# fuxiao0719/PanopticNeRF

Measured on AMD Instinct MI355X. Metric: Msamples/sec (coarse+fine), KITTI-360 1408x376, higher is better.
Workload: dtype bf16

## Files before the change

### include/pnr.h

```cpp
#ifndef PNR_H
#define PNR_H
#include <stdint.h>

#ifdef __cplusplus
extern "C" {
#endif

#define PNR_OK 0
#define PNR_EINVAL (-1)
#define PNR_EHIP (-2)
#define PNR_ENODEV (-3)

#define PNR_PREC_BF16 0
#define PNR_PREC_FP32 1

int pnr_version(void);
const char* pnr_last_error(void);
int pnr_device_check(int dev, char* buf_host, int buflen);

int pnr_stratified(const float* rays, int64_t n_rays, int n_samples, int lindisp,
                   const float* t_rand, float* z_out, void* stream);

int pnr_points(const float* rays, const float* z, int64_t n_rays, int n_samples, float* pts_out,
               void* stream);

int pnr_embed(const float* x, int64_t n, int L, float* out, void* stream);

typedef struct pnr_mlp_desc {
    int32_t D, W, skip;
    int32_t xyz_L, dir_L;
    int32_t n_sem, n_inst, head_W;
    int32_t precision;
    int32_t plan;
    int32_t head_tap;
    int32_t head_depth;
    int32_t schedule;
    int32_t clk_probe[2];
    int32_t flags;
} pnr_mlp_desc;

#define PNR_MLP_SOFTMAX 1
#define PNR_MLP_WG_CAP(n) (((n) & 0x1FF) << 16)
#define PNR_MLP_TRACE 0x7A00

typedef struct pnr_mlp_params_host {
    const float* const* pts_w; const float* const* pts_b;
    const float* alpha_w; const float* alpha_b;
    const float* feature_w; const float* feature_b;
    const float* views_w; const float* views_b;
    const float* rgb_w; const float* rgb_b;
    const float* sem0_w; const float* sem0_b; const float* sem1_w; const float* sem1_b;
    const float* inst0_w; const float* inst0_b; const float* inst1_w; const float* inst1_b;
} pnr_mlp_params_host;

int64_t pnr_mlp_packed_bytes(const pnr_mlp_desc* desc);
int pnr_mlp_pack(const pnr_mlp_desc* desc, const pnr_mlp_params_host* params, void* packed_host);

int64_t pnr_mlp_pack_workspace_bytes(const pnr_mlp_desc* desc, int backward);
int pnr_mlp_pack_device(const pnr_mlp_desc* desc, const pnr_mlp_params_host* params_dev, int backward,
                        void* workspace, void* packed, void* stream);
int pnr_mlp_repack_device(const pnr_mlp_desc* desc, const pnr_mlp_params_host* params_dev, int backward,
                          void* workspace, void* packed, void* stream);

int pnr_mlp_forward(const pnr_mlp_desc* desc, const void* packed, const float* rays, const float* z,
                    int64_t n_rays, int n_samples, float* raw, int64_t raw_stride_s,
                    int64_t raw_stride_c, void* stream);

int pnr_mlp_fused_plan(const pnr_mlp_desc* desc);
int64_t pnr_mlp_forward_composite_workspace_bytes(const pnr_mlp_desc* desc, int64_t n_rays, int n_samples, int want_weights);
int pnr_mlp_forward_composite(const pnr_mlp_desc* desc, const void* packed, const float* rays, const float* z,
                              int64_t n_rays, int n_samples, const int32_t* label_sem, const int32_t* label_inst,
                              int white_bkgd, float* rgb, float* depth, float* acc, float* weights, float* sem,
                              float* inst, float* fix_sem, float* fix_inst, void* workspace, void* stream);

int pnr_mlp_forward_tiles(const pnr_mlp_desc* desc, const void* packed, const float* rays, const float* z, int64_t n_rays,
                          int n_samples, void* workspace, void* stream);
int pnr_composite_combine(const pnr_mlp_desc* desc, const void* workspace, const float* z, int64_t n_rays, int n_samples,
                          const int32_t* label_sem, const int32_t* label_inst, int white_bkgd, float* rgb, float* depth,
                          float* acc, float* weights, float* sem, float* inst, float* fix_sem, float* fix_inst, void* stream);

int pnr_mlp_query(const pnr_mlp_desc* desc, const void* packed, const float* points, int64_t n_points,
                  float* sigma, int32_t* sem_label, int32_t* inst_label, int32_t* panoptic, const int32_t* is_thing,
                  float* sem_logits, float* inst_logits, int64_t logit_stride, void* stream);
int pnr_mlp_query_supported(const pnr_mlp_desc* desc);

int pnr_mlp_train_layout(const pnr_mlp_desc* desc, int64_t n_samples, int64_t* acts_off_host ,
                         int64_t* dys_off_host );
int pnr_mlp_forward_train(const pnr_mlp_desc* desc, const void* packed, const float* rays, const float* z,
                          int64_t n_rays, int n_samples, float* raw, int64_t raw_stride_s,
                          int64_t raw_stride_c, void* acts, void* stream);
int64_t pnr_mlp_bwd_packed_bytes(const pnr_mlp_desc* desc);
int pnr_mlp_pack_bwd(const pnr_mlp_desc* desc, const pnr_mlp_params_host* params, void* packed_host);
int pnr_mlp_backward(const pnr_mlp_desc* desc, const void* packed_bwd, const float* d_raw, const void* acts,
                     void* dys, int64_t n_rays, int n_samples, void* stream);

int64_t pnr_mlp_wgrad_workspace_bytes(const pnr_mlp_desc* desc, int64_t n_samples);
int pnr_mlp_wgrad(const pnr_mlp_desc* desc, const void* acts, const void* dys, int64_t n_samples,
                  const pnr_mlp_params_host* grads_dev, void* workspace, void* stream);

int64_t pnr_mlp_fp32_acts_floats(const pnr_mlp_desc* desc, int64_t n_samples);
int64_t pnr_mlp_backward_fp32_workspace_bytes(const pnr_mlp_desc* desc, int64_t n_samples);
int pnr_mlp_forward_train_fp32(const pnr_mlp_desc* desc, const pnr_mlp_params_host* params_dev, const float* rays,
                               const float* z, int64_t n_rays, int n_samples, float* raw, int64_t raw_stride_s,
                               int64_t raw_stride_c, float* acts, void* stream);
int pnr_mlp_backward_fp32(const pnr_mlp_desc* desc, const pnr_mlp_params_host* params_dev, const float* d_raw,
                          int64_t d_raw_stride_c, const float* acts, int64_t n_rays, int n_samples,
                          const pnr_mlp_params_host* grads_dev, void* workspace, void* stream);

int pnr_composite(const float* raw, int64_t raw_stride_s, int64_t raw_stride_c, const float* z,
                  const float* rays, const float* noise, const int32_t* label_sem,
                  const int32_t* label_inst, int64_t n_rays, int n_samples, int n_sem, int n_inst,
                  int sem_mode, int white_bkgd, float* rgb, float* depth, float* acc, float* weights,
                  float* sem, float* inst, float* fix_sem, float* fix_inst, void* stream);

int pnr_composite_backward(const float* raw, int64_t raw_stride_c, const float* z, const float* rays,
                           const float* noise, int64_t n_rays, int n_samples, int n_sem, int n_inst,
                           const float* g_rgb, const float* g_depth, const float* g_acc, const float* g_sem,
                           const float* g_inst, const float* g_weights, float* d_raw, void* stream);

int pnr_composite_backward2(const float* raw, int64_t raw_stride_c, const float* z, const float* rays,
                            const float* noise, int64_t n_rays, int n_samples, int n_sem, int n_inst,
                            const float* g_rgb, const float* g_depth, const float* g_acc, const float* g_sem,
                            const float* g_inst, const float* g_weights, const int32_t* label_sem,
                            const int32_t* label_inst, const float* g_fix_sem, const float* g_fix_inst,
// ... 174 lines not shown
```

### panopticnerf_amd/_lib.py

```python
import ctypes
import os

_HERE = os.path.dirname(os.path.abspath(__file__))
LIB_PATH = os.environ.get("PNR_LIB_PATH") or os.path.join(_HERE, "libpnr.so")

c_f = ctypes.c_void_p
c_i64 = ctypes.c_int64
c_int = ctypes.c_int

PREC_BF16, PREC_FP32 = 0, 1
MLP_SOFTMAX, MLP_TRACE = 1, 0x7A00
CAMERA_PINHOLE, CAMERA_FISHEYE, CAMERA_EQUIRECT = 0, 1, 3
TAG_PIXEL, TAG_FRAME = 16, 17
SAMPLE_POOLED, SAMPLE_FRAME = 0, 1


class LossCfg(ctypes.Structure):
    _fields_ = [("w_rgb", ctypes.c_float), ("w_depth", ctypes.c_float), ("w_sem", ctypes.c_float),
                ("w_fix_sem", ctypes.c_float), ("w_inst", ctypes.c_float), ("w_fix_inst", ctypes.c_float),
                ("depth_l2", ctypes.c_int32), ("fix_eps", ctypes.c_float), ("maps_are_prob", ctypes.c_int32)]


class MlpDesc(ctypes.Structure):
    _fields_ = [("D", ctypes.c_int32), ("W", ctypes.c_int32), ("skip", ctypes.c_int32),
                ("xyz_L", ctypes.c_int32), ("dir_L", ctypes.c_int32),
                ("n_sem", ctypes.c_int32), ("n_inst", ctypes.c_int32), ("head_W", ctypes.c_int32),
                ("precision", ctypes.c_int32), ("plan", ctypes.c_int32), ("head_tap", ctypes.c_int32),
                ("head_depth", ctypes.c_int32), ("schedule", ctypes.c_int32), ("clk_probe", ctypes.c_int32 * 2), ("flags", ctypes.c_int32)]


class RngDesc(ctypes.Structure):
    _fields_ = [("call", ctypes.c_void_p), ("ray_base", ctypes.c_int64), ("tag", ctypes.c_int32), ("scale", ctypes.c_float)]


class Frame(ctypes.Structure):
    _fields_ = [("model", ctypes.c_int32), ("width", ctypes.c_int32), ("height", ctypes.c_int32), ("cam", ctypes.c_float * 7),
                ("c2w", ctypes.c_float * 12), ("near_", ctypes.c_float), ("far_", ctypes.c_float), ("n_valid", ctypes.c_int64),
                ("valid_pix", ctypes.c_uint64), ("rgb", ctypes.c_uint64), ("depth", ctypes.c_uint64), ("sem", ctypes.c_uint64),
                ("inst", ctypes.c_uint64)]


_fp = ctypes.POINTER(ctypes.c_float)
_fpp = ctypes.POINTER(_fp)


class MlpParamsHost(ctypes.Structure):
    _fields_ = [("pts_w", _fpp), ("pts_b", _fpp),
                ("alpha_w", _fp), ("alpha_b", _fp), ("feature_w", _fp), ("feature_b", _fp),
                ("views_w", _fp), ("views_b", _fp), ("rgb_w", _fp), ("rgb_b", _fp),
                ("sem0_w", _fp), ("sem0_b", _fp), ("sem1_w", _fp), ("sem1_b", _fp),
                ("inst0_w", _fp), ("inst0_b", _fp), ("inst1_w", _fp), ("inst1_b", _fp)]


SIGNATURES = {
    "pnr_version": (c_int, []),
    "pnr_last_error": (ctypes.c_char_p, []),
    "pnr_device_check": (c_int, [c_int, ctypes.c_char_p, c_int]),
    "pnr_stratified": (c_int, [c_f, c_i64, c_int, c_int, c_f, c_f, c_f]),
    "pnr_points": (c_int, [c_f, c_f, c_i64, c_int, c_f, c_f]),
    "pnr_embed": (c_int, [c_f, c_i64, c_int, c_f, c_f]),
    "pnr_mlp_packed_bytes": (c_i64, [ctypes.POINTER(MlpDesc)]),
    "pnr_mlp_pack": (c_int, [ctypes.POINTER(MlpDesc), ctypes.POINTER(MlpParamsHost), ctypes.c_void_p]),
    "pnr_mlp_pack_workspace_bytes": (c_i64, [ctypes.POINTER(MlpDesc), c_int]),
    "pnr_mlp_pack_device": (c_int, [ctypes.POINTER(MlpDesc), ctypes.POINTER(MlpParamsHost), c_int, c_f, c_f, c_f]),
    "pnr_mlp_repack_device": (c_int, [ctypes.POINTER(MlpDesc), ctypes.POINTER(MlpParamsHost), c_int, c_f, c_f, c_f]),
    "pnr_mlp_forward": (c_int, [ctypes.POINTER(MlpDesc), c_f, c_f, c_f, c_i64, c_int, c_f, c_i64, c_i64, c_f]),
    "pnr_mlp_train_layout": (c_int, [ctypes.POINTER(MlpDesc), c_i64, ctypes.POINTER(c_i64), ctypes.POINTER(c_i64)]),
    "pnr_mlp_forward_train": (c_int, [ctypes.POINTER(MlpDesc), c_f, c_f, c_f, c_i64, c_int, c_f, c_i64, c_i64, c_f, c_f]),
    "pnr_mlp_bwd_packed_bytes": (c_i64, [ctypes.POINTER(MlpDesc)]),
    "pnr_mlp_pack_bwd": (c_int, [ctypes.POINTER(MlpDesc), ctypes.POINTER(MlpParamsHost), ctypes.c_void_p]),
    "pnr_mlp_backward": (c_int, [ctypes.POINTER(MlpDesc), c_f, c_f, c_f, c_f, c_i64, c_int, c_f]),
    "pnr_mlp_wgrad_workspace_bytes": (c_i64, [ctypes.POINTER(MlpDesc), c_i64]),
    "pnr_mlp_wgrad": (c_int, [ctypes.POINTER(MlpDesc), c_f, c_f, c_i64, ctypes.POINTER(MlpParamsHost), c_f, c_f]),
    "pnr_mlp_fp32_acts_floats": (c_i64, [ctypes.POINTER(MlpDesc), c_i64]),
    "pnr_mlp_backward_fp32_workspace_bytes": (c_i64, [ctypes.POINTER(MlpDesc), c_i64]),
    "pnr_mlp_forward_train_fp32": (c_int, [ctypes.POINTER(MlpDesc), ctypes.POINTER(MlpParamsHost), c_f, c_f, c_i64, c_int, c_f, c_i64,
                                           c_i64, c_f, c_f]),
    "pnr_mlp_backward_fp32": (c_int, [ctypes.POINTER(MlpDesc), ctypes.POINTER(MlpParamsHost), c_f, c_i64, c_f, c_i64, c_int,
                                      ctypes.POINTER(MlpParamsHost), c_f, c_f]),
    "pnr_mlp_fused_plan": (c_int, [ctypes.POINTER(MlpDesc)]),
    "pnr_mlp_forward_composite_workspace_bytes": (c_i64, [ctypes.POINTER(MlpDesc), c_i64, c_int, c_int]),
    "pnr_mlp_forward_composite": (c_int, [ctypes.POINTER(MlpDesc), c_f, c_f, c_f, c_i64, c_int, c_f, c_f, c_int,
                                          c_f, c_f, c_f, c_f, c_f, c_f, c_f, c_f, c_f, c_f]),
    "pnr_composite": (c_int, [c_f, c_i64, c_i64, c_f, c_f, c_f, c_f, c_f, c_i64, c_int, c_int, c_int, c_int,
                              c_int, c_f, c_f, c_f, c_f, c_f, c_f, c_f, c_f, c_f]),
    "pnr_composite_backward": (c_int, [c_f, c_i64, c_f, c_f, c_f, c_i64, c_int, c_int, c_int,
                                       c_f, c_f, c_f, c_f, c_f, c_f, c_f, c_f]),
    "pnr_composite_backward2": (c_int, [c_f, c_i64, c_f, c_f, c_f, c_i64, c_int, c_int, c_int,
                                        c_f, c_f, c_f, c_f, c_f, c_f, c_f, c_f, c_f, c_f, c_f, c_f, c_f, c_f]),
    "pnr_composite_backward3": (c_int, [c_f, c_i64, c_f, c_f, c_f, c_i64, c_int, c_int, c_int, c_int,
                                        c_f, c_f, c_f, c_f, c_f, c_f, c_f, c_f, c_f, c_f, c_f, c_f, c_f, c_f]),
    "pnr_losses_workspace_bytes": (c_i64, [c_i64]),
    "pnr_losses": (c_int, [ctypes.POINTER(LossCfg), c_i64, c_int, c_int] + [c_f] * 19),
    "pnr_ce3d_workspace_bytes": (c_i64, [c_i64]),
# ... 83 lines not shown
```

### panopticnerf_amd/csrc/pnr_composite.hip

```cpp
#include "pnr_composite_dev.h"

struct CompositeArgs {
    const float* raw; int64_t stride_s, stride_c;
    const float* z; const float* rays; const float* noise;
    const int32_t* label_sem; const int32_t* label_inst;
    int64_t R; int N, C, K, sem_mode, white_bkgd;
    float *rgb, *depth, *acc, *weights, *sem, *inst, *fix_sem, *fix_inst;
    int use_hist;
};

#ifndef CMP_GRID_PER_CU
#define CMP_GRID_PER_CU 8
#endif
#ifndef CMP_UB
#define CMP_UB 8
#endif

__device__ __forceinline__ float dot4(const f4& w, const f4& v)
{
    return fmaf(w.v[3], v.v[3], fmaf(w.v[2], v.v[2], fmaf(w.v[1], v.v[1], w.v[0] * v.v[0])));
}

template <bool CH_MAJOR, int SUB, bool SOFTMAX, class... Rng>
__global__ __launch_bounds__(256) void k_composite(CompositeArgs a, const Rng... rng)
// ... 221 lines not shown
            group_sum_batch<L, CMP2_UB>(r);
            if (writer) store_rows<CMP2_UB>(a, ray, q0, nq, r, accv);
        }
    }
}

static int composite_impl(const float* raw, int64_t raw_stride_s, int64_t raw_stride_c, const float* z, const float* rays,
                          const float* noise, const PnrRngDev* rng, const int32_t* label_sem, const int32_t* label_inst, int64_t n_rays,
                          int n_samples, int n_sem, int n_inst, int sem_mode, int white_bkgd, float* rgb, float* depth, float* acc,
                          float* weights, float* sem, float* inst, float* fix_sem, float* fix_inst, void* stream)
{
    PNR_REQUIRE(n_rays <= 0 || (raw && z && rays), "pnr_composite: null pointer");
    PNR_REQUIRE(n_samples >= 4 && n_samples <= 256 && (n_samples % 4) == 0,
                "pnr_composite: n_samples=%d must be a multiple of 4 in [4,256]", n_samples);
    PNR_REQUIRE(n_sem >= 0 && n_inst >= 0 && (sem_mode == 0 || sem_mode == 1), "pnr_composite: bad field sizes");
    PNR_REQUIRE((((uintptr_t)z) & 15) == 0, "pnr_composite: z must be 16-byte aligned");
    PNR_REQUIRE(!weights || (((uintptr_t)weights) & 15) == 0, "pnr_composite: weights must be 16-byte aligned");
    PNR_REQUIRE((((uintptr_t)noise) & 15) == 0 && (((uintptr_t)label_sem) & 15) == 0 && (((uintptr_t)label_inst) & 15) == 0,
                "pnr_composite: noise / label arrays must be 16-byte aligned");
    if (n_rays <= 0) return PNR_OK;
    CompositeArgs a;
    a.raw = raw; a.stride_s = raw_stride_s; a.stride_c = raw_stride_c; a.z = z; a.rays = rays; a.noise = noise;
    a.label_sem = label_sem; a.label_inst = label_inst; a.R = n_rays; a.N = n_samples; a.C = n_sem; a.K = n_inst;
    a.sem_mode = sem_mode; a.white_bkgd = white_bkgd; a.rgb = rgb; a.depth = depth; a.acc = acc; a.weights = weights;
    a.sem = sem; a.inst = inst; a.fix_sem = fix_sem; a.fix_inst = fix_inst;
    const bool want_fix = (fix_sem && label_sem && n_sem) || (fix_inst && label_inst && n_inst);
    const bool ch_major = raw_stride_s == 1 && (raw_stride_c % 4) == 0 && (((uintptr_t)raw) & 15) == 0;
    hipStream_t st = (hipStream_t)stream;
    auto hist_bytes = [&](int rpw) { return (size_t)4 * rpw * (n_sem + n_inst) * sizeof(uint32_t); };
    auto grid_for = [&](int rpw) { return pnr_grid_cap(((n_rays + rpw - 1) / rpw + 3) / 4, CMP_GRID_PER_CU); };
    if (ch_major && n_samples > 32 && n_samples <= 64 && (!want_fix || hist_bytes(8) <= 48 * 1024)) {
        a.use_hist = want_fix ? 1 : 0;
        const size_t lds = want_fix ? hist_bytes(8) : 0;
        composite_dispatch<8>(8, true, sem_mode, rng, [&](auto L, auto, auto SM, const auto&... r) {
            hipLaunchKernelGGL((k_composite2<decltype(L)::value, 2, decltype(SM)::value, std::decay_t<decltype(r)>...>), dim3(grid_for(8)), dim3(256),
                               lds, st, a, r...);
        });
        PNR_CHECK_LAUNCH("pnr_composite");
        return PNR_OK;
    }
    int sub = 1;
    while (sub < n_samples / 4) sub <<= 1;
    const int rpw = 64 / sub;
    a.use_hist = (want_fix && hist_bytes(rpw) <= 48 * 1024) ? 1 : 0;
    const size_t lds = a.use_hist ? hist_bytes(rpw) : 0;
    composite_dispatch<1, 2, 4, 8, 16, 32, 64>(sub, ch_major, sem_mode, rng, [&](auto S, auto CH, auto SM, const auto&... r) {
        hipLaunchKernelGGL((k_composite<decltype(CH)::value, decltype(S)::value, decltype(SM)::value, std::decay_t<decltype(r)>...>),
                           dim3(grid_for(rpw)), dim3(256), lds, st, a, r...);
    });
    PNR_CHECK_LAUNCH("pnr_composite");
    return PNR_OK;
}

PNR_EXPORT int pnr_composite(const float* raw, int64_t raw_stride_s, int64_t raw_stride_c, const float* z,
                             const float* rays, const float* noise, const int32_t* label_sem,
                             const int32_t* label_inst, int64_t n_rays, int n_samples, int n_sem, int n_inst,
                             int sem_mode, int white_bkgd, float* rgb, float* depth, float* acc, float* weights,
                             float* sem, float* inst, float* fix_sem, float* fix_inst, void* stream)
{
    return composite_impl(raw, raw_stride_s, raw_stride_c, z, rays, noise, nullptr, label_sem, label_inst, n_rays, n_samples, n_sem, n_inst,
                          sem_mode, white_bkgd, rgb, depth, acc, weights, sem, inst, fix_sem, fix_inst, stream);
}

PNR_EXPORT int pnr_composite_rng(const float* raw, int64_t raw_stride_s, int64_t raw_stride_c, const float* z, const float* rays,
                                 const pnr_rng* noise_host, const int32_t* label_sem, const int32_t* label_inst, int64_t n_rays,
                                 int n_samples, int n_sem, int n_inst, int sem_mode, int white_bkgd, float* rgb, float* depth, float* acc,
                                 float* weights, float* sem, float* inst, float* fix_sem, float* fix_inst, void* stream)
{
    PnrRngDev rng;
    const int rc = pnr_rng_check(noise_host, n_rays < 0 ? 0 : n_rays, "pnr_composite_rng", &rng);
    if (rc) return rc;
    PNR_REQUIRE(n_rays <= 0 || (raw_stride_s == 1 && (raw_stride_c % 4) == 0 && (((uintptr_t)raw) & 15) == 0),
                "pnr_composite_rng: channel-major, 16-byte aligned raw images only");
    return composite_impl(raw, raw_stride_s, raw_stride_c, z, rays, nullptr, &rng, label_sem, label_inst, n_rays, n_samples, n_sem, n_inst,
                          sem_mode, white_bkgd, rgb, depth, acc, weights, sem, inst, fix_sem, fix_inst, stream);
}

struct CombineArgs {
    const float* rec; int rec_floats; const float4* ps; const float* z; const int32_t* lab_s; const int32_t* lab_i;
    int64_t R; int N, C, K, white_bkgd;
    float *rgb, *depth, *acc, *weights, *sem, *inst, *fix_sem, *fix_inst;
};

template <bool LOGITS>
__global__ __launch_bounds__(256) void k_composite_combine(CombineArgs a)
{
    __shared__ uint32_t hist_all[4][128];
    const int lane = threadIdx.x & 63, wv = threadIdx.x >> 6;
    const int64_t ray = ((int64_t)blockIdx.x * blockDim.x + threadIdx.x) >> 6;
    if (ray >= a.R) return;
    const int N = a.N, T = N >> 5, RF = a.rec_floats, C = a.C, K = a.K, CK = C + K;
    const float* __restrict__ rec = a.rec + ray * T * RF;
    const float4* __restrict__ ps = a.ps + ray * N;
    const float* __restrict__ zr = a.z + ray * N;
    const bool want_s = a.lab_s && a.fix_sem && C, want_i = a.lab_i && a.fix_inst && K;
    const int32_t* __restrict__ lsr = want_s ? a.lab_s + ray * N : nullptr;
    const int32_t* __restrict__ lir = want_i ? a.lab_i + ray * N : nullptr;
    float q[8];
#pragma unroll
    for (int k = 0; k < 8; ++k) q[k] = k < T ? rec[k * RF] : 1.0f;
    float4 pv[4];
    float zv[4];
    int lsv[4], liv[4];
#pragma unroll
    for (int j = 0; j < 4; ++j) {
        const int i = lane + 64 * j;
        const bool in = i < N;
        pv[j] = in ? ps[i] : float4{0.0f, 0.0f, 0.0f, 0.0f};
        zv[j] = in ? zr[i] : 0.0f;
        lsv[j] = (in && want_s) ? lsr[i] : -1;
        liv[j] = (in && want_i) ? lir[i] : -1;
    }
    float lg[2][8];
#pragma unroll
    for (int h = 0; h < 2; ++h)
#pragma unroll
        for (int k = 0; k < 8; ++k) lg[h][k] = (LOGITS && k < T && lane + 64 * h < CK) ? rec[k * RF + PNR_FUSE_REC_LOGITS + lane + 64 * h] : 0.0f;
    float Tk[8];
    float t = 1.0f;
#pragma unroll
    for (int k = 0; k < 8; ++k) {
        Tk[k] = t;
        if (k < T) t *= q[k];
    }
    uint32_t* hist = hist_all[wv];
    if (want_s || want_i) hist_zero<64>(hist, lane, CK);
    float r5[5] = {0.0f, 0.0f, 0.0f, 0.0f, 0.0f};
#pragma unroll
    for (int j = 0; j < 4; ++j) {
        const int i = lane + 64 * j;
        if (i < N) {
            const float4 p = pv[j];
            float tk = Tk[0];
#pragma unroll
            for (int k = 1; k < 8; ++k) tk = (i >> 5) == k ? Tk[k] : tk;
            const float w = tk * p.x;
            r5[0] += w;
            r5[1] = fmaf(w, zv[j], r5[1]);
            r5[2] = fmaf(w, sigmoid_of(p.y), r5[2]);
            r5[3] = fmaf(w, sigmoid_of(p.z), r5[3]);
            r5[4] = fmaf(w, sigmoid_of(p.w), r5[4]);
            if (a.weights) a.weights[ray * N + i] = w;
            if (want_s || want_i) hist_add(hist, w, want_s, lsv[j], C, want_i, liv[j], K);
        }
    }
    group_sum_batch<64, 5>(r5);
    if (lane == 0) {
        if (a.acc) a.acc[ray] = r5[0];
        if (a.depth) a.depth[ray] = r5[1];
    }
    if (lane < 3 && a.rgb) {
        const float v = lane == 0 ? r5[2] : lane == 1 ? r5[3] : r5[4];
        a.rgb[ray * 3 + lane] = a.white_bkgd ? v + (1.0f - r5[0]) : v;
    }
#pragma unroll
    for (int h = 0; h < 2; ++h) {
        const int c = lane + 64 * h;
        if (c >= CK) continue;
        if constexpr (LOGITS) {
            float v = 0.0f;
#pragma unroll
            for (int k = 0; k < 8; ++k) if (k < T) v = fmaf(Tk[k], lg[h][k], v);
            if (c < C) { if (a.sem) a.sem[ray * C + c] = v; }
            else if (a.inst) a.inst[ray * K + (c - C)] = v;
        }
        if (c < C) { if (want_s) a.fix_sem[ray * C + c] = hist_read(hist, c); }
        else if (want_i) a.fix_inst[ray * K + (c - C)] = hist_read(hist, c);
    }
}

int pnr_composite_combine_launch(const float* rec, int rec_floats, bool logit_sums, const float4* ps, const float* z,
                                 const int32_t* label_sem, const int32_t* label_inst, int64_t R, int N, int C, int K, int white_bkgd,
                                 float* rgb, float* depth, float* acc, float* weights, float* sem, float* inst, float* fix_sem,
                                 float* fix_inst, hipStream_t st)
{
    CombineArgs a;
    a.rec = rec; a.rec_floats = rec_floats; a.ps = ps; a.z = z; a.lab_s = label_sem; a.lab_i = label_inst;
    a.R = R; a.N = N; a.C = C; a.K = K; a.white_bkgd = white_bkgd;
    a.rgb = rgb; a.depth = depth; a.acc = acc; a.weights = weights; a.sem = sem; a.inst = inst; a.fix_sem = fix_sem; a.fix_inst = fix_inst;
    const int64_t blocks = (R + 3) / 4;
    if (logit_sums) hipLaunchKernelGGL(k_composite_combine<true>, dim3((unsigned)blocks), dim3(256), 0, st, a);
    else hipLaunchKernelGGL(k_composite_combine<false>, dim3((unsigned)blocks), dim3(256), 0, st, a);
    PNR_CHECK_LAUNCH("pnr_mlp_forward_composite (combine)");
    return PNR_OK;
}
```

### panopticnerf_amd/csrc/pnr_mlp.hip

```cpp
#include <stdlib.h>
#include <string.h>

#include "pnr_mlp_plan.h"

int pnr_mlp_validate(const pnr_mlp_desc* d);

#include "pnr_mlp_core.h"
#include "pnr_mlp_pp.h"
#ifndef PNR_FUSE_TRANSPOSED
#define PNR_FUSE_TRANSPOSED 1
#endif
#include "pnr_mlp_fuse.h"
#include "pnr_mlp_tt.h"
#define PNR_QUERY_MAX_POINTS (((int64_t)1 << 31) - 4096)
#ifndef PNR_TRAIN_TILES_EXPERIMENT
#define PNR_TRAIN_TILES_EXPERIMENT 0
#endif
template <int PREC, int TILES, class CTX, int KIND, int NA, int NB, int NFB_OUT, int MODE, int NOUT>
__device__ __forceinline__ void layer_regs(CTX& c, const uint32_t (&inA)[TILES][NA],
                                           const uint32_t (&inB)[TILES][NB > 0 ? NB : 1],
                                           uint32_t (&out)[TILES][NOUT], uint16_t* save = nullptr,
                                           const int* srow = nullptr)
{
    constexpr int RPB = PrecT<PREC>::RPB;
// ... 717 lines not shown
    return PNR_OK;
}


static inline unsigned long long* clk_probe_of(const pnr_mlp_desc* d)
{
    return (unsigned long long*)(uintptr_t)(((uint64_t)(uint32_t)d->clk_probe[1] << 32) | (uint64_t)(uint32_t)d->clk_probe[0]);
}

static void mlp_args_fill(MlpArgs& a, const pnr_mlp_desc* desc, const PnrPlan& plan, const void* packed)
{
    memset(&a, 0, sizeof(a));
    a.data = (const uint8_t*)packed + plan.data_off;
    a.table = (const pnr_chunk_entry*)((const uint8_t*)packed + plan.table_off);
    a.n_chunks = (int)plan.chunks.size();
    a.slot_bytes = plan.max_chunk_frags * PNR_FRAG_BYTES;
    a.D = desc->D; a.skip = desc->skip; a.n_sem = desc->n_sem; a.n_inst = desc->n_inst;
    a.head_tap = desc->head_tap; a.head_depth = desc->head_depth == 1 ? 1 : 2;
    a.clk = clk_probe_of(desc);
#if PNR_TRACE
    if (const char* e = getenv("PNR_TRACE_PTR")) a.trace = (unsigned long long*)strtoull(e, nullptr, 0);
#endif
}

static int mlp_forward_impl(const pnr_mlp_desc* desc, const void* packed, const float* rays, const float* z,
                            int64_t n_rays, int n_samples, float* raw, int64_t raw_stride_s, int64_t raw_stride_c,
                            void* acts, void* stream)
{
    int rc = pnr_mlp_validate(desc);
    if (rc != PNR_OK) return rc;
    PNR_REQUIRE(n_rays >= 0 && n_samples >= 1, "pnr_mlp_forward: bad size");
    if (n_rays == 0) return PNR_OK;
    PNR_REQUIRE(packed && rays && z && raw, "pnr_mlp_forward: null pointer");
    PNR_REQUIRE(n_rays * (int64_t)n_samples < ((int64_t)1 << 31) - 4096, "pnr_mlp_forward: R*N=%lld exceeds 2^31",
                (long long)(n_rays * n_samples));
    PNR_REQUIRE((((uintptr_t)rays) & 15) == 0 && (((uintptr_t)packed) & 15) == 0 && (((uintptr_t)acts) & 15) == 0,
                "pnr_mlp_forward: rays / packed / acts must be 16-byte aligned");
    PNR_REQUIRE(!acts || desc->precision == PNR_PREC_BF16, "pnr_mlp_forward_train: the training path is bf16 only");
    PNR_REQUIRE(desc->plan != 4, "pnr_mlp_forward: a plan-4 (field) image is for pnr_mlp_query only");
    PNR_REQUIRE(desc->plan == 0, "pnr_mlp_forward: plan=%d images are for pnr_mlp_forward_composite only", desc->plan);
    PnrPlan plan;
    pnr_build_plan(*desc, plan);
    MlpArgs a;
    mlp_args_fill(a, desc, plan, packed);
    a.rays = rays; a.z = z; a.S = (int)(n_rays * n_samples); a.N = n_samples;
    pnr_set_div_magic(n_samples, a.n_magic, a.n_shift);
    a.raw = raw; a.ss = raw_stride_s; a.sc = raw_stride_c;
    a.acts = (uint16_t*)acts;
    if (acts) pnr_train_layout(*desc, a.S, a.acts_off, a.dys_off, a.gate_off);
    hipStream_t st = (hipStream_t)stream;
    if (desc->precision == PNR_PREC_BF16) {
        if (desc->schedule != 1 && !acts)
            return desc->W == 256 ? launch_mlp_pp<256, false>(a, st) : launch_mlp_pp<128, false>(a, st);
        if (desc->schedule == 2 && acts)
            return desc->W == 256 ? launch_mlp_pp<256, true>(a, st) : launch_mlp_pp<128, true>(a, st);
#if PNR_TRAIN_TILES_EXPERIMENT
        if (acts && desc->schedule == 3 && desc->W == 256) return launch_mlp<PNR_PREC_BF16, 256, 2, 4, 1, true>(a, st);
        if (acts && desc->schedule == 4 && desc->W == 256) {
            PNR_REQUIRE(a.S % 384 == 0, "schedule 4 (experiment): S must be a multiple of 384");
            return launch_mlp<PNR_PREC_BF16, 256, 3, 4, 1, true>(a, st);
        }
#endif
        if (acts)
            return desc->W == 256 ? launch_mlp<PNR_PREC_BF16, 256, 1, 8, 2, true>(a, st)
                                  : launch_mlp<PNR_PREC_BF16, 128, 1, 8, 2, true>(a, st);
        return desc->W == 256 ? launch_mlp<PNR_PREC_BF16, 256, 1, 8, 2>(a, st) : launch_mlp<PNR_PREC_BF16, 128, 1, 8, 2>(a, st);
    }
    return desc->W == 256 ? launch_mlp<PNR_PREC_FP32, 256, 1, 4, 1>(a, st) : launch_mlp<PNR_PREC_FP32, 128, 1, 4, 1>(a, st);
}

PNR_EXPORT int pnr_mlp_forward(const pnr_mlp_desc* desc, const void* packed, const float* rays, const float* z,
                               int64_t n_rays, int n_samples, float* raw, int64_t raw_stride_s,
                               int64_t raw_stride_c, void* stream)
{
    return mlp_forward_impl(desc, packed, rays, z, n_rays, n_samples, raw, raw_stride_s, raw_stride_c, nullptr, stream);
}

#define PNR_RAY_AUX_BYTES 128
#define PNR_TT_SAVE_REGION (352 * 1024)
static bool pnr_tt_save_proto() { static const bool on = getenv("PNR_TT_SAVE_PROTO") != nullptr; return on; }
int pnr_composite_combine_launch(const float* rec, int rec_floats, bool logit_sums, const float4* ps, const float* z,
                                 const int32_t* label_sem, const int32_t* label_inst, int64_t R, int N, int C, int K, int white_bkgd,
                                 float* rgb, float* depth, float* acc, float* weights, float* sem, float* inst, float* fix_sem,
                                 float* fix_inst, hipStream_t st);

static int record_floats(const pnr_mlp_desc& d)
{
    return d.plan == 3 ? pnr_fuse_record_floats(0, 0) : pnr_fuse_record_floats(d.n_sem, d.n_inst);
}

PNR_EXPORT int64_t pnr_mlp_forward_composite_workspace_bytes(const pnr_mlp_desc* desc, int64_t n_rays, int n_samples, int want_weights)
{
    (void)want_weights;
    if (pnr_mlp_validate(desc) != PNR_OK || n_rays < 0 || n_samples < 32 || (n_samples & 31)) return -1;
    const int64_t S = n_rays * n_samples, tiles = (S + 255) / 256 * 8;
    if (desc->plan == 3) return tiles * record_floats(*desc) * 4 + S * 16 + 256;
    return tiles * pnr_fuse_record_floats(desc->n_sem, desc->n_inst) * 4 + S * 16 + 256 + PNR_RAY_AUX_BYTES + n_rays * PNR_RAY_AUX_BYTES +
           (pnr_tt_save_proto() ? tiles / 8 * 4 * PNR_TT_SAVE_REGION + 4096 : 0);
}

__global__ void __launch_bounds__(256) k_ray_aux(const float* __restrict__ rays, int64_t R, uint32_t* __restrict__ aux)
{
    const int64_t i = (int64_t)blockIdx.x * 256 + threadIdx.x;
    if (i >= 2 * R) return;
    const int64_t ray = i >> 1;
    const int hi = (int)(i & 1);
    const float dx = rays[ray * 8 + 3], dy = rays[ray * 8 + 4], dz = rays[ray * 8 + 5];
    const float nrm = sqrtf(__fadd_rn(__fadd_rn(__fmul_rn(dx, dx), __fmul_rn(dy, dy)), __fmul_rn(dz, dz)));
    uint32_t ed[8];
    embed_lane<PNR_PREC_BF16, 2, 16, 8>(dx / nrm, dy / nrm, dz / nrm, hi, ed);
    uint4* o = reinterpret_cast<uint4*>(aux + i * 16);
    o[0] = make_uint4(ed[0], ed[1], ed[2], ed[3]);
    o[1] = make_uint4(ed[4], ed[5], ed[6], ed[7]);
    o[2] = make_uint4(__float_as_uint(nrm), 0u, 0u, 0u);
}

static int fused_mlp_launch(const pnr_mlp_desc* desc, const void* packed, const float* rays, const float* z, int64_t n_rays,
                            int n_samples, void* workspace, void* stream, MlpArgs& a)
{
    int rc = pnr_mlp_validate(desc);
    if (rc != PNR_OK) return rc;
    PNR_REQUIRE(desc->precision == PNR_PREC_BF16, "pnr_mlp_forward_composite: bf16 only");
    PNR_REQUIRE(desc->plan != 4, "pnr_mlp_forward_composite: a plan-4 (field) image is for pnr_mlp_query only");
    PNR_REQUIRE(n_rays >= 1 && n_samples >= 32 && n_samples <= 256 && (n_samples & 31) == 0,
                "pnr_mlp_forward_composite: n_samples=%d must be a multiple of 32 in [32,256]", n_samples);
    PNR_REQUIRE(desc->n_sem + desc->n_inst <= 128, "pnr_mlp_forward_composite: n_sem + n_inst <= 128");
    PNR_REQUIRE(packed && rays && z && workspace, "pnr_mlp_forward_composite: null pointer");
    PNR_REQUIRE(n_rays * (int64_t)n_samples < ((int64_t)1 << 31) - 4096, "pnr_mlp_forward_composite: R*N exceeds 2^31");
    PNR_REQUIRE((((uintptr_t)rays | (uintptr_t)packed | (uintptr_t)workspace) & 15) == 0,
                "pnr_mlp_forward_composite: rays / packed / workspace must be 16-byte aligned");
    PnrPlan plan;
    pnr_build_plan(*desc, plan);
    mlp_args_fill(a, desc, plan, packed);
    a.rays = rays; a.z = z; a.S = (int)(n_rays * n_samples); a.N = n_samples;
    pnr_set_div_magic(n_samples, a.n_magic, a.n_shift);
    a.rec_floats = record_floats(*desc);
    a.rec = (float*)workspace;
    const int64_t tiles = ((int64_t)a.S + 255) / 256 * 8;
    a.ps = (float4*)(a.rec + tiles * a.rec_floats);
    hipStream_t st = (hipStream_t)stream;
    const bool softmax = (desc->flags & PNR_MLP_SOFTMAX) && desc->n_sem + desc->n_inst > 0;
    if (desc->plan == 3)
        return desc->W == 256 ? launch_mlp_pp<256, false, true, 0, true>(a, st) : launch_mlp_pp<128, false, true, 0, true>(a, st);
    if (desc->plan == 2) {
        PnrTTArgs t;
        memset(&t, 0, sizeof(t));
        t.image = a.data; t.rays = rays; t.z = z; t.S = a.S; t.N = a.N; t.n_magic = a.n_magic; t.n_shift = a.n_shift;
        t.rec = a.rec; t.rec_floats = a.rec_floats; t.ps = a.ps; t.n_sem = a.n_sem; t.n_inst = a.n_inst; t.clk = a.clk;
        PNR_REQUIRE(n_rays < ((int64_t)1 << 24), "pnr_mlp_forward_composite: the two-tile kernel addresses 2^24 rays per launch");
        uint32_t* aux = (uint32_t*)(((uintptr_t)((uint8_t*)a.ps + (int64_t)a.S * 16 + 256) + PNR_RAY_AUX_BYTES - 1)
                                    & ~(uintptr_t)(PNR_RAY_AUX_BYTES - 1));
        k_ray_aux<<<dim3((unsigned)((2 * n_rays + 255) / 256)), dim3(256), 0, st>>>(rays, n_rays, aux);
        t.aux = aux;
        t.n_wg = (desc->flags >> 16) & 0x1FF;
        if (pnr_tt_save_proto()) t.save = (void*)(((uintptr_t)((uint8_t*)aux + n_rays * PNR_RAY_AUX_BYTES) + 4095) & ~(uintptr_t)4095);
        const bool trace = (desc->flags & 0xFF00) == PNR_MLP_TRACE;
        return pnr_mlp_tt_launch(t, (desc->n_sem + 31) / 32, (desc->n_inst + 31) / 32, a.head_depth, a.head_tap, softmax, st, trace,
                                 trace ? ((desc->flags >> 4) & 7) : 0);
    }
    if (desc->plan == 1) {
        const int nbs = (desc->n_sem + 31) / 32, nbi = (desc->n_inst + 31) / 32;
        switch (4 * nbs + nbi + (softmax ? 16 : 0)) {
        case 4: return launch_mlp_pp<256, false, true, 4>(a, st);
        case 5: return launch_mlp_pp<256, false, true, 5>(a, st);
        case 8: return launch_mlp_pp<256, false, true, 8>(a, st);
        case 9: return launch_mlp_pp<256, false, true, 9>(a, st);
        case 20: return launch_mlp_pp<256, false, true, 20>(a, st);
        case 21: return launch_mlp_pp<256, false, true, 21>(a, st);
        case 24: return launch_mlp_pp<256, false, true, 24>(a, st);
        case 25: return launch_mlp_pp<256, false, true, 25>(a, st);
        default: PNR_REQUIRE(false, "pnr_mlp_forward_composite: no plan-1 kernel for %d + %d logit blocks", nbs, nbi);
        }
    }
    PNR_REQUIRE(!softmax, "pnr_mlp_forward_composite: softmax compositing needs the plan-1 image (pnr_mlp_fused_plan >= 1, desc.plan = 1)");
    return desc->W == 256 ? launch_mlp_pp<256, false, true>(a, st) : launch_mlp_pp<128, false, true>(a, st);
}

PNR_EXPORT int pnr_mlp_forward_tiles(const pnr_mlp_desc* desc, const void* packed, const float* rays, const float* z, int64_t n_rays,
                                     int n_samples, void* workspace, void* stream)
{
    PNR_REQUIRE(n_rays >= 0, "pnr_mlp_forward_tiles: bad size");
    if (n_rays == 0) return PNR_OK;
    MlpArgs a;
    return fused_mlp_launch(desc, packed, rays, z, n_rays, n_samples, workspace, stream, a);
}

PNR_EXPORT int pnr_composite_combine(const pnr_mlp_desc* desc, const void* workspace, const float* z, int64_t n_rays, int n_samples,
                                     const int32_t* label_sem, const int32_t* label_inst, int white_bkgd, float* rgb, float* depth,
                                     float* acc, float* weights, float* sem, float* inst, float* fix_sem, float* fix_inst, void* stream)
{
    int rc = pnr_mlp_validate(desc);
    if (rc != PNR_OK) return rc;
    PNR_REQUIRE(n_rays >= 0 && n_samples >= 32 && n_samples <= 256 && (n_samples & 31) == 0, "pnr_composite_combine: bad size");
    if (n_rays == 0) return PNR_OK;
    PNR_REQUIRE(workspace && z, "pnr_composite_combine: null pointer");
    PNR_REQUIRE(desc->plan != 4, "pnr_composite_combine: a plan-4 (field) image has no compositing workspace");
    PNR_REQUIRE((!fix_sem || label_sem) && (!fix_inst || label_inst), "pnr_composite_combine: fix_* outputs need their labels");
    PNR_REQUIRE(desc->plan != 3 || (!rgb && !sem && !inst), "pnr_composite_combine: a plan-3 (sigma-only) workspace has no rgb, semantic "
                "or instance maps: pass null for them");
    const int rf = record_floats(*desc);
    const int64_t tiles = (n_rays * n_samples + 255) / 256 * 8;
    const float* rec = (const float*)workspace;
    return pnr_composite_combine_launch(rec, rf, desc->plan != 3, (const float4*)(rec + tiles * rf), z, fix_sem ? label_sem : nullptr,
                                        fix_inst ? label_inst : nullptr, n_rays, n_samples, desc->n_sem, desc->n_inst, white_bkgd,
                                        rgb, depth, acc, weights, sem, inst, fix_sem, fix_inst, (hipStream_t)stream);
}

PNR_EXPORT int pnr_mlp_forward_composite(const pnr_mlp_desc* desc, const void* packed, const float* rays, const float* z,
                                         int64_t n_rays, int n_samples, const int32_t* label_sem, const int32_t* label_inst,
                                         int white_bkgd, float* rgb, float* depth, float* acc, float* weights, float* sem,
                                         float* inst, float* fix_sem, float* fix_inst, void* workspace, void* stream)
{
    PNR_REQUIRE(n_rays >= 0, "pnr_mlp_forward_composite: bad size");
    if (n_rays == 0) return PNR_OK;
    PNR_REQUIRE((!fix_sem || label_sem) && (!fix_inst || label_inst), "pnr_mlp_forward_composite: fix_* outputs need their labels");
    PNR_REQUIRE(!desc || desc->plan != 3 || (!rgb && !sem && !inst), "pnr_mlp_forward_composite: a plan-3 (sigma-only) image has no "
                "rgb, semantic or instance maps: pass null for them");
    MlpArgs a;
    int rc = fused_mlp_launch(desc, packed, rays, z, n_rays, n_samples, workspace, stream, a);
    if (rc != PNR_OK) return rc;
    return pnr_composite_combine_launch(a.rec, a.rec_floats, desc->plan != 3, a.ps, z, fix_sem ? label_sem : nullptr, fix_inst ? label_inst : nullptr,
                                        n_rays, n_samples, desc->n_sem, desc->n_inst, white_bkgd, rgb, depth, acc, weights, sem, inst,
                                        fix_sem, fix_inst, (hipStream_t)stream);
}

PNR_EXPORT int pnr_mlp_forward_train(const pnr_mlp_desc* desc, const void* packed, const float* rays, const float* z,
                                     int64_t n_rays, int n_samples, float* raw, int64_t raw_stride_s,
                                     int64_t raw_stride_c, void* acts, void* stream)
{
    PNR_REQUIRE(acts || n_rays == 0, "pnr_mlp_forward_train: acts is null");
    return mlp_forward_impl(desc, packed, rays, z, n_rays, n_samples, raw, raw_stride_s, raw_stride_c, acts, stream);
}

PNR_EXPORT int pnr_mlp_train_layout(const pnr_mlp_desc* desc, int64_t n_samples, int64_t* acts_off_host,
                                    int64_t* dys_off_host)
{
    int rc = pnr_mlp_validate(desc);
    if (rc != PNR_OK) return rc;
    PNR_REQUIRE(acts_off_host && dys_off_host && n_samples >= 0, "pnr_mlp_train_layout: bad arguments");
    int64_t a[24], d[24];
    pnr_train_layout(*desc, n_samples, a, d);
    memcpy(acts_off_host, a, sizeof(int64_t) * (size_t)(desc->D + 7));
    memcpy(dys_off_host, d, sizeof(int64_t) * (size_t)(desc->D + 8));
    return PNR_OK;
}

struct FieldArgs {
    MlpArgs m;
    const float* pts;
    float* sigma;
    int32_t* sem_label; int32_t* inst_label; int32_t* panoptic;
    const int32_t* is_thing;
    float* sem_logits; float* inst_logits; int64_t lstride;
    int run_sem, run_inst;
};

template <class CTX, int NA, class EPI>
__device__ __forceinline__ void pp_field_out(CTX& c, u32x4 (&A)[CTX::P], const uint32_t (&in)[NA], int n_out, EPI&& epi)
{
    using CH = PPChunk<1, NA, 0>;
    const uint32_t dummy[1] = {0};
    const int nfb = (n_out + 31) >> 5;
#pragma unroll 1
    for (int fb = 0; fb < nfb; ++fb) {
        f32x16 acc[1];
        CH::prologue(c.frag_addr(), c.bias_addr(), A, acc);
        CH::mma(c.frag_addr(), A, in, dummy, acc, [&](auto... k) { if constexpr (sizeof...(k) == 0) { c.stamp(6); c.barrier(); c.stamp(2); } else c.stamp(k...); });
        c.m_done();
        c.refill_begin();
        c.refill_one();
        epi(fb, acc[0]);
        c.refill_rest();
        c.advance();
    }
}

struct FieldBest { float v; int i; };
__device__ __forceinline__ void field_best_merge(FieldBest& b, int hi)
{
    const auto pv = __builtin_amdgcn_permlane32_swap(__float_as_uint(b.v), __float_as_uint(b.v), false, false);
    const auto pi = __builtin_amdgcn_permlane32_swap((uint32_t)b.i, (uint32_t)b.i, false, false);
    const float ov = __uint_as_float(hi ? pv[0] : pv[1]);
    const int oi = (int)(hi ? pi[0] : pi[1]);
    if (ov > b.v || (ov == b.v && oi < b.i)) { b.v = ov; b.i = oi; }
    if (b.i == 0x7fffffff) b.i = 0;
}

template <int W, bool HEADS>
__global__ __launch_bounds__(512, 2) void k_mlp_pp_field(const FieldArgs fa)
{
    constexpr int WAVES = 8;
    using CTX = CtxPP<WAVES>;
    extern __shared__ __attribute__((aligned(16))) char smem[];
    constexpr int NFB = W / 32, HFB = W / 64;
    constexpr int HR = NFB * 8, GR = HFB * 8, GXR = 16;
    const MlpArgs& a = fa.m;
    CTX c = pp_ctx<WAVES>(a, smem);
    unsigned long long clk_c0, clk_r0;
    pp_begin(c, clk_c0, clk_r0);
    const int n = c.lane & 31;

    uint32_t dummy[1] = {0};
    u32x4 A[CTX::P];
    struct PointIn { float x, y, z; };
    auto fetch_point = [&](int grp) {
        const int s = (grp * WAVES + c.wave) * 32 + n;
// ... 119 lines not shown
```

### panopticnerf_amd/csrc/pnr_mlp_pack.cpp

```cpp
#include <math.h>
#include <string.h>

#include <vector>

#include "pnr_common.h"
#include "pnr_mlp_layout.h"
#include "pnr_mlp_plan.h"
#include "pnr_mlp_tt.h"

int pnr_mlp_validate(const pnr_mlp_desc* d)
{
    PNR_REQUIRE(d, "pnr_mlp: null desc");
    PNR_REQUIRE(d->W == 256 || d->W == 128, "pnr_mlp: W=%d unsupported (128 or 256)", d->W);
    PNR_REQUIRE(d->D >= 2 && d->D <= 16, "pnr_mlp: D=%d outside [2,16]", d->D);
    PNR_REQUIRE(d->skip >= -1 && d->skip < d->D - 1, "pnr_mlp: skip=%d must be -1 or < D-1", d->skip);
    PNR_REQUIRE(d->xyz_L >= 0 && d->xyz_L <= 10, "pnr_mlp: xyz_L=%d outside [0,10]", d->xyz_L);
    PNR_REQUIRE(d->dir_L >= 0 && d->dir_L <= 4, "pnr_mlp: dir_L=%d outside [0,4]", d->dir_L);
    PNR_REQUIRE(d->n_sem >= 0 && d->n_sem <= 256 && d->n_inst >= 0 && d->n_inst <= 256,
                "pnr_mlp: n_sem/n_inst outside [0,256]");
    PNR_REQUIRE((d->n_sem == 0 && d->n_inst == 0) || d->head_W == d->W / 2,
                "pnr_mlp: head_W=%d must equal W/2=%d", d->head_W, d->W / 2);
    PNR_REQUIRE(d->precision == PNR_PREC_BF16 || d->precision == PNR_PREC_FP32, "pnr_mlp: bad precision %d",
                d->precision);
    PNR_REQUIRE(d->head_tap == 0 || d->head_tap == 1, "pnr_mlp: head_tap=%d must be 0 (trunk output) or 1 (feature)", d->head_tap);
    PNR_REQUIRE(d->head_depth >= 0 && d->head_depth <= 2, "pnr_mlp: head_depth=%d must be 1 or 2", d->head_depth);
#ifndef PNR_TRAIN_TILES_EXPERIMENT
#define PNR_TRAIN_TILES_EXPERIMENT 0
#endif
    PNR_REQUIRE(d->schedule >= 0 && d->schedule <= (PNR_TRAIN_TILES_EXPERIMENT ? 6 : 2), "pnr_mlp: schedule=%d must be 0 (default), 1 (lock-step) or 2 (ping-pong)", d->schedule);
    PNR_REQUIRE(d->plan == 0 || (d->plan == 1 && pnr_plan1_supported(*d)) || (d->plan == 2 && pnr_plan2_supported(*d)) ||
                (d->plan == 3 && pnr_plan3_supported(*d)) || (d->plan == 4 && pnr_plan4_supported(*d)),
                "pnr_mlp: plan=%d is not available for this geometry (ask pnr_mlp_fused_plan; plans 3 and 4: bf16 only)", d->plan);
    const uint32_t trace = (uint32_t)d->flags & 0xFF00u;
    PNR_REQUIRE(((uint32_t)d->flags & ~(uint32_t)(PNR_MLP_SOFTMAX | 0xFF70u | PNR_MLP_WG_CAP(0x1FF))) == 0 && (trace == 0 || trace == PNR_MLP_TRACE) &&
                (trace != 0 || ((uint32_t)d->flags & 0x70u) == 0),
                "pnr_mlp: unknown bits in flags=0x%x (zero-initialise pnr_mlp_desc; PNR_MLP_* are the defined bits)", (unsigned)d->flags);
    PNR_REQUIRE(((uint32_t)d->clk_probe[0] & 15u) == 0, "pnr_mlp: clk_probe=0x%08x%08x is not a 16-byte aligned device address "
                "(zero-initialise pnr_mlp_desc; clk_probe is a diagnostics field, 0 = off)", (unsigned)d->clk_probe[1], (unsigned)d->clk_probe[0]);
    PNR_REQUIRE(trace == 0 || (d->clk_probe[0] | d->clk_probe[1]) != 0, "pnr_mlp: PNR_MLP_TRACE needs clk_probe");
    return PNR_OK;
}

PNR_EXPORT int pnr_mlp_fused_plan(const pnr_mlp_desc* desc)
{
    if (!desc) return 0;
    pnr_mlp_desc d = *desc;
    d.plan = 0;
    if (pnr_mlp_validate(&d) != PNR_OK) return 0;
    if ((d.flags & PNR_MLP_SOFTMAX) && d.n_sem + d.n_inst > 0)
        return pnr_plan2_supported(d) ? 2 : pnr_plan1_supported(d) ? 1 : 0;
    return pnr_plan2_supported(d) ? 2 : pnr_plan1_supported(d) ? 1 : 0;
}

PNR_EXPORT int pnr_mlp_query_supported(const pnr_mlp_desc* desc)
{
    if (!desc) return 0;
    pnr_mlp_desc d = *desc;
    d.plan = 0;
    if (pnr_mlp_validate(&d) != PNR_OK) return 0;
    return pnr_plan4_supported(d);
}

static int bwd_validate(const pnr_mlp_desc* d)
{
    int rc = pnr_mlp_validate(d);
    if (rc != PNR_OK) return rc;
    PNR_REQUIRE(d->plan == 0, "pnr_mlp backward: plan must be 0");
    PNR_REQUIRE(d->precision == PNR_PREC_BF16, "pnr_mlp backward: bf16 only");
    PNR_REQUIRE(d->n_sem <= PNR_BWD_OUT_SLOTS && d->n_inst <= PNR_BWD_OUT_SLOTS,
                "pnr_mlp backward: n_sem / n_inst must be <= %d", PNR_BWD_OUT_SLOTS);
    return PNR_OK;
}

static int check_params(const pnr_mlp_desc* desc, const pnr_mlp_params_host* p, bool bias)
{
    PNR_REQUIRE(p, "pnr_mlp_pack: null params");
    if (desc->plan == 3) {
        PNR_REQUIRE(p->pts_w && p->alpha_w && (!bias || (p->pts_b && p->alpha_b)), "pnr_mlp_pack: missing trunk or alpha_linear parameter");
        return PNR_OK;
    }
    if (desc->plan == 4) {
        const bool feat = desc->head_tap == 1 && (desc->n_sem || desc->n_inst);
        PNR_REQUIRE(p->pts_w && p->alpha_w && (!bias || (p->pts_b && p->alpha_b)), "pnr_mlp_pack: missing trunk or alpha_linear parameter");
        PNR_REQUIRE(!feat || (p->feature_w && (!bias || p->feature_b)), "pnr_mlp_pack: missing feature_linear parameter");
    } else {
    PNR_REQUIRE(p->pts_w && p->alpha_w && p->feature_w && p->views_w && p->rgb_w, "pnr_mlp_pack: missing trunk parameter");
    if (bias) PNR_REQUIRE(p->pts_b && p->alpha_b && p->feature_b && p->views_b && p->rgb_b, "pnr_mlp_pack: missing trunk bias");
    }
    const bool deep = pnr_head_depth(*desc) == 2;
    if (desc->n_sem) PNR_REQUIRE((!deep || p->sem0_w) && p->sem1_w && (!bias || ((!deep || p->sem0_b) && p->sem1_b)), "pnr_mlp_pack: missing semantic head");
    if (desc->n_inst) PNR_REQUIRE((!deep || p->inst0_w) && p->inst1_w && (!bias || ((!deep || p->inst0_b) && p->inst1_b)), "pnr_mlp_pack: missing instance head");
    return PNR_OK;
}

struct Image {
    pnr_pack_header hdr;
    std::vector<pnr_chunk_entry> table;
    std::vector<PnrFragDesc> frags;
    size_t table_off, data_off, total_bytes;
};

static PnrFragDesc zero_desc()
{
    PnrFragDesc f;
    memset(&f, 0, sizeof(f));
    return f;
}

static void fill_header(Image& im, const pnr_mlp_desc& d, int version, size_t n_chunks, int max_frags, size_t table_off,
                        size_t data_off, size_t total)
{
    memset(&im.hdr, 0, sizeof(im.hdr));
    im.hdr.magic = PNR_PACK_MAGIC;
    im.hdr.version = (uint32_t)version;
    im.hdr.n_chunks = (uint32_t)n_chunks;
    im.hdr.max_chunk_frags = (uint32_t)max_frags;
    im.hdr.table_off = (uint32_t)table_off;
// ... 273 lines not shown
```

### panopticnerf_amd/csrc/pnr_sampling.hip

```cpp
#include "pnr_common.h"
#include "pnr_philox.h"
#include <stdlib.h>
#include <string.h>

#pragma clang fp contract(off)

__device__ __forceinline__ float pnr_linspace01(int i, int N)
{
    if (N <= 1) return 0.0f;
    const float step = 1.0f / (float)(N - 1);
    if (i < N / 2) return step * (float)i;
    return fmaf(-step, (float)(N - 1 - i), 1.0f);
}

__device__ __forceinline__ float strat_z(float nr, float fr, int i, int N, int lindisp)
{
    const float t = pnr_linspace01(i, N);
    const float omt = 1.0f - t;
    if (!lindisp) {
        const float a = nr * omt, b = fr * t;
        return a + b;
    }
    const float a = (1.0f / nr) * omt, b = (1.0f / fr) * t;
    return 1.0f / (a + b);
// ... 3 lines not shown
{
    const float zi = strat_z(nr, fr, i, N, lindisp);
    if (!t) return zi;
    const float z0 = strat_z(nr, fr, 0, N, lindisp), zl = strat_z(nr, fr, N - 1, N, lindisp);
    const float lo = (i == 0) ? z0 : 0.5f * (zi + strat_z(nr, fr, i - 1, N, lindisp));
    const float up = (i == N - 1) ? zl : 0.5f * (strat_z(nr, fr, i + 1, N, lindisp) + zi);
    const float w = up - lo;
    const float m = w * *t;
    return lo + m;
}

template <class... Rng>
__global__ __launch_bounds__(256) void k_stratified(const float* __restrict__ rays, int64_t R, int N,
                                                     int lindisp, const float* __restrict__ t_rand,
                                                     float* __restrict__ z_out, const Rng... rng)
{
    constexpr bool RNG = sizeof...(Rng) > 0;
    PnrRngKey key;
    if constexpr (RNG) key = pnr_rng_key(rng...);
    const int64_t total = R * N;
    for (int64_t s = (int64_t)blockIdx.x * blockDim.x + threadIdx.x; s < total;
         s += (int64_t)gridDim.x * blockDim.x) {
        const int64_t r = s / N;
        const int i = (int)(s - r * N);
        if constexpr (RNG) {
            const float t = pnr_rng_uniform_at(key, (uint32_t)r, i);
            z_out[s] = strat_sample(rays[r * 8 + 6], rays[r * 8 + 7], i, N, lindisp, &t);
        } else {
            z_out[s] = strat_sample(rays[r * 8 + 6], rays[r * 8 + 7], i, N, lindisp, t_rand ? t_rand + s : nullptr);
        }
    }
}

__global__ __launch_bounds__(256) void k_points(const float* __restrict__ rays, const float* __restrict__ z,
                                                 int64_t R, int N, float* __restrict__ pts)
{
    const int64_t total = R * N * 3;
    for (int64_t e = (int64_t)blockIdx.x * blockDim.x + threadIdx.x; e < total;
         e += (int64_t)gridDim.x * blockDim.x) {
        const int64_t s = e / 3;
        const int a = (int)(e - s * 3);
        const int64_t r = s / N;
        const float m = rays[r * 8 + 3 + a] * z[s];
        pts[e] = rays[r * 8 + a] + m;
    }
}

__global__ __launch_bounds__(256) void k_embed(const float* __restrict__ x, int64_t n, int L,
                                                float* __restrict__ out)
{
    const int E = 3 + 6 * L;
    const int64_t total = n * E;
    for (int64_t e = (int64_t)blockIdx.x * blockDim.x + threadIdx.x; e < total;
         e += (int64_t)gridDim.x * blockDim.x) {
        const int64_t s = e / E;
        const int c = (int)(e - s * E);
        float v;
        if (c < 3) {
            v = x[s * 3 + c];
        } else {
            const int k = (c - 3) / 6, j = (c - 3) - 6 * k;
            const int a = j % 3;
            const float arg = x[s * 3 + a] * ldexpf(1.0f, k);
            v = (j < 3) ? sinf(arg) : cosf(arg);
        }
        out[e] = v;
    }
}

template <class F>
__device__ __forceinline__ int label_hit(float zz, int cnt, F interval)
{
    int best = -1;
    float bt = 0.0f;
    for (int h = 0; h < cnt; ++h) {
        float ti, to;
        interval(h, ti, to);
        if (ti <= zz && zz <= to && (best < 0 || ti < bt)) {
            best = h;
            bt = ti;
        }
    }
    return best;
}

struct PdfLabelArgs {
    const float* hit_t; const int32_t* hit_box; const int32_t* hit_count; int max_hits; const int32_t* box_ids;
    int32_t* label_sem; int32_t* label_inst;
};
#define PDF_MAXC 256
#define PDF_MAXT 512
template <int MAXC, int MAXT, bool RNG = false>
__device__ __forceinline__ void sample_pdf_body(const float* __restrict__ z, const float* __restrict__ weights,
                                                    const float* __restrict__ u, int64_t R, int Nc, int Nf,
                                                    float* __restrict__ zs_out, int32_t* __restrict__ inds_out,
                                                    float* __restrict__ zfine_out, const PdfLabelArgs lab,
                                                    const PnrRngDev& rng = PnrRngDev{})
{
    PnrRngKey key;
    if constexpr (RNG) key = pnr_rng_key(rng);
    __shared__ float s_z[MAXC], s_w[MAXC], s_pdf[MAXC], s_cdf[MAXC], s_bins[MAXC];
    __shared__ float s_sort[MAXT], s_out[MAXT];
    __shared__ float s_total, s_part[32];
    const int lane = threadIdx.x;
    const int nb = Nc - 1, nw = Nc - 2, Nt = Nc + Nf;
    const bool short4 = nw >= 4 && nw < 8;
    int P = 1;
    while (P < Nt) P <<= 1;
    auto labels = [&](int64_t r, const float* sorted) {
        if (!lab.label_sem) return;
        const int mh = lab.max_hits;
        const int cnt = lab.hit_count[r] < mh ? lab.hit_count[r] : mh;
        for (int i = lane; i < Nt; i += 64) {
            const int best = label_hit(sorted[i], cnt, [&](int h, float& ti, float& to) {
                ti = lab.hit_t[(r * mh + h) * 2];
                to = lab.hit_t[(r * mh + h) * 2 + 1];
            });
            int ls = -1, li = -1;
            if (best >= 0) {
                const int m = lab.hit_box[r * mh + best];
                ls = lab.box_ids[m * 2];
                li = lab.box_ids[m * 2 + 1];
            }
            lab.label_sem[r * Nt + i] = ls;
            lab.label_inst[r * Nt + i] = li;
        }
    };
    for (int64_t r = blockIdx.x; r < R; r += gridDim.x) {
        for (int i = lane; i < Nc; i += 64) {
            s_z[i] = z[r * Nc + i];
            s_w[i] = weights[r * Nc + i];
        }
        __syncthreads();
        for (int k = lane; k < nb; k += 64) s_bins[k] = 0.5f * (s_z[k + 1] + s_z[k]);
        if (lane < 32) {
            const int k = lane >> 3, l = lane & 7, nv = nw / 8, groups = nv / 4;
            float pacc = 0.0f;
            for (int g = 0; g < groups; ++g) pacc = pacc + (s_w[(g * 4 + k) * 8 + l + 1] + 1e-5f);
            if (k == 0)
                for (int v = groups * 4; v < nv; ++v) pacc = pacc + (s_w[v * 8 + l + 1] + 1e-5f);
            if (short4 && lane < 3) pacc = pacc + (s_w[lane + 2] + 1e-5f);
            s_part[lane] = pacc;
        }
        __syncthreads();
        if (lane == 0) {
            const int nv = nw / 8;
            float total = 0.0f;
            for (int j = nv * 8; j < nw; j = (short4 && j == 0) ? 4 : j + 1) total = total + (s_w[j + 1] + 1e-5f);
            for (int l = 0; l < 8; ++l) {
                float p0 = s_part[l];
                p0 = p0 + s_part[8 + l]; p0 = p0 + s_part[16 + l]; p0 = p0 + s_part[24 + l];
                total = total + p0;
            }
            s_total = total;
        }
        __syncthreads();
        const float total = s_total;
        for (int j = lane; j < nw; j += 64) s_pdf[j] = (s_w[j + 1] + 1e-5f) / total;
        __syncthreads();
        const float pl = lane < nw ? s_pdf[lane < nw ? lane : 0] : 0.0f;
        double c = (double)pl;
        bool exact = nw <= 64 && __all(pl == 0.0f || pl >= 0x1p-28f);
        if (exact) {
#pragma unroll
            for (int d = 1; d < 64; d <<= 1) {
                const double o = __shfl_up(c, d, 64);
                if (lane >= d) c += o;
            }
            exact = __shfl(c, 63, 64) < 1.999;
        }
        if (exact) {
            if (lane == 0) s_cdf[0] = 0.0f;
            if (lane < nw) s_cdf[lane + 1] = (float)c;
        } else if (lane == 0) {
            double c = 0.0;
            s_cdf[0] = 0.0f;
            for (int j = 0; j < nw; ++j) {
                c += (double)s_pdf[j];
                s_cdf[j + 1] = (float)c;
            }
        }
        __syncthreads();
        for (int i = lane; i < Nf; i += 64) {
            float uu;
            if constexpr (RNG) uu = pnr_rng_uniform_at(key, (uint32_t)r, i);
            else uu = u ? u[r * Nf + i] : pnr_linspace01(i, Nf);
            int lo = 0, hi = nb;
            while (lo < hi) {
                const int mid = (lo + hi) >> 1;
                if (s_cdf[mid] <= uu) lo = mid + 1; else hi = mid;
            }
            const int inds = lo;
            const int below = inds - 1 > 0 ? inds - 1 : 0;
            const int above = inds < nb - 1 ? inds : nb - 1;
            float denom = s_cdf[above] - s_cdf[below];
            if (denom < 1e-5f) denom = 1.0f;
            const float t = (uu - s_cdf[below]) / denom;
            const float span = s_bins[above] - s_bins[below];
            const float m = t * span;
            const float zs = s_bins[below] + m;
            if (zs_out) zs_out[r * Nf + i] = zs;
            if (inds_out) inds_out[r * Nf + i] = inds;
            s_sort[Nc + i] = zs;
        }
        if (zfine_out) {
            __syncthreads();
            bool asc = true;
            for (int i = lane; i + 1 < Nf; i += 64) asc = asc && (s_sort[Nc + i] <= s_sort[Nc + i + 1]);
// ... 153 lines not shown
                for (int j = 0; j < nw; ++j) {
                    cc += (double)s_pdf[j];
                    s_cdf[j + 1] = (float)cc;
                }
            }
        }
        __syncthreads();
        bool asc = lane + 1 >= Nc || zl <= zn;
        for (int i = lane; i < Nf; i += 64) {
            const float uu = pnr_linspace01(i, Nf);
            int pos = 0;
            for (int st = topc; st >= 1; st >>= 1) {
                const int p = pos + st, q = p <= nb ? p : nb;
                pos = (p <= nb && s_cdf[q - 1] <= uu) ? p : pos;
            }
            const int inds = pos;
            const int below = inds - 1 > 0 ? inds - 1 : 0;
            const int above = inds < nb - 1 ? inds : nb - 1;
            const float cb = s_cdf[below];
            float denom = s_cdf[above] - cb;
            if (denom < 1e-5f) denom = 1.0f;
            const float t = (uu - cb) / denom;
            const float bb = s_bins[below];
            const float span = s_bins[above] - bb;
            const float m = t * span;
            const float zs = bb + m;
            s_zs[i] = zs;
        }
        __syncthreads();
        for (int i = lane; i + 1 < Nf; i += 64) asc = asc && (s_zs[i] <= s_zs[i + 1]);
        if (__all(asc)) {
            if (lane < Nc) {
                int pos = 0;
                for (int st = topf; st >= 1; st >>= 1) {
                    const int p = pos + st, q = p <= Nf ? p : Nf;
                    pos = (p <= Nf && s_zs[q - 1] < zl) ? p : pos;
                }
                s_out[lane + pos] = zl;
            }
            for (int j = lane; j < Nf; j += 64) {
                const float v = s_zs[j];
                int pos = 0;
                for (int st = topc; st >= 1; st >>= 1) {
                    const int p = pos + st, q = p <= Nc ? p : Nc;
                    pos = (p <= Nc && s_z[q - 1] <= v) ? p : pos;
                }
                s_out[j + pos] = v;
            }
            __syncthreads();
        } else {
            int P = 1;
            while (P < Nt) P <<= 1;
            pdf_bitonic_fallback(s_out, s_z, s_zs, Nc, Nf, P, lane);
        }
        float* __restrict__ zo = zfine_out + r * Nt;
        for (int i0 = 0; i0 < Nt; i0 += 256) {
            float zz[4];
            int best[4], ls[4], li[4];
            float bt[4];
#pragma unroll
            for (int k = 0; k < 4; ++k) {
                const int i = i0 + lane + 64 * k;
                zz[k] = i < Nt ? s_out[i < Nt ? i : 0] : 0.0f;
                best[k] = -1; ls[k] = -1; li[k] = -1; bt[k] = 0.0f;
                if (i < Nt) zo[i] = zz[k];
            }
            if (lab.label_sem) {
                for (int h = 0; h < cnt; ++h) {
                    const float ti = __int_as_float(__builtin_amdgcn_readlane(__float_as_int(h_ti), h));
                    const float to = __int_as_float(__builtin_amdgcn_readlane(__float_as_int(h_to), h));
                    const int hs = __builtin_amdgcn_readlane(h_ls, h), hi2 = __builtin_amdgcn_readlane(h_li, h);
#pragma unroll
                    for (int k = 0; k < 4; ++k) {
                        const bool take = ti <= zz[k] && zz[k] <= to && (best[k] < 0 || ti < bt[k]);
                        best[k] = take ? h : best[k];
                        bt[k] = take ? ti : bt[k];
                        ls[k] = take ? hs : ls[k];
                        li[k] = take ? hi2 : li[k];
                    }
                }
#pragma unroll
                for (int k = 0; k < 4; ++k) {
                    const int i = i0 + lane + 64 * k;
                    if (i < Nt) {
                        lab.label_sem[r * Nt + i] = ls[k];
                        lab.label_inst[r * Nt + i] = li[k];
                    }
                }
            }
        }
        __syncthreads();
    }
}

__global__ __launch_bounds__(64) __attribute__((amdgpu_waves_per_eu(8, 8)))
void k_sample_pdf(const float* __restrict__ z, const float* __restrict__ weights, const float* __restrict__ u, int64_t R, int Nc, int Nf,
                  float* __restrict__ zs_out, int32_t* __restrict__ inds_out, float* __restrict__ zfine_out, const PdfLabelArgs lab)
{
    sample_pdf_body<64, 256>(z, weights, u, R, Nc, Nf, zs_out, inds_out, zfine_out, lab);
}
__global__ __launch_bounds__(64)
void k_sample_pdf_big(const float* __restrict__ z, const float* __restrict__ weights, const float* __restrict__ u, int64_t R, int Nc, int Nf,
                      float* __restrict__ zs_out, int32_t* __restrict__ inds_out, float* __restrict__ zfine_out, const PdfLabelArgs lab)
{
    sample_pdf_body<PDF_MAXC, PDF_MAXT>(z, weights, u, R, Nc, Nf, zs_out, inds_out, zfine_out, lab);
}
__global__ __launch_bounds__(64) __attribute__((amdgpu_waves_per_eu(8, 8)))
void k_sample_pdf_rng(const float* __restrict__ z, const float* __restrict__ weights, int64_t R, int Nc, int Nf, float* __restrict__ zs_out,
                      int32_t* __restrict__ inds_out, float* __restrict__ zfine_out, const PdfLabelArgs lab, const PnrRngDev rng)
{
    sample_pdf_body<64, 256, true>(z, weights, nullptr, R, Nc, Nf, zs_out, inds_out, zfine_out, lab, rng);
}
__global__ __launch_bounds__(64)
void k_sample_pdf_big_rng(const float* __restrict__ z, const float* __restrict__ weights, int64_t R, int Nc, int Nf,
                          float* __restrict__ zs_out, int32_t* __restrict__ inds_out, float* __restrict__ zfine_out, const PdfLabelArgs lab,
                          const PnrRngDev rng)
{
    sample_pdf_body<PDF_MAXC, PDF_MAXT, true>(z, weights, nullptr, R, Nc, Nf, zs_out, inds_out, zfine_out, lab, rng);
}

__global__ __launch_bounds__(256) void k_bbox_hits(const float* __restrict__ rays, int64_t R,
                                                    const float* __restrict__ box, int M, int max_hits,
                                                    float* __restrict__ hit_t, int32_t* __restrict__ hit_box,
                                                    int32_t* __restrict__ hit_count)
{
    for (int64_t r = (int64_t)blockIdx.x * blockDim.x + threadIdx.x; r < R;
         r += (int64_t)gridDim.x * blockDim.x) {
        const float o0 = rays[r * 8 + 0], o1 = rays[r * 8 + 1], o2 = rays[r * 8 + 2];
        const float d0 = rays[r * 8 + 3], d1 = rays[r * 8 + 4], d2 = rays[r * 8 + 5];
        const float nr = rays[r * 8 + 6], fr = rays[r * 8 + 7];
        for (int h = 0; h < max_hits; ++h) {
            hit_box[r * max_hits + h] = -1;
            hit_t[(r * max_hits + h) * 2 + 0] = 0.0f;
            hit_t[(r * max_hits + h) * 2 + 1] = 0.0f;
        }
        int cnt = 0;
        for (int m = 0; m < M; ++m) {
            const float* b = box + m * 15;
            const float p0 = o0 - b[0], p1 = o1 - b[1], p2 = o2 - b[2];
            float tmin = nr, tmax = fr;
#pragma unroll
            for (int a = 0; a < 3; ++a) {
                const float r0 = b[3 + 3 * a], r1 = b[4 + 3 * a], r2 = b[5 + 3 * a];
                const float ol = (r0 * p0 + r1 * p1) + r2 * p2;
                const float dl = (r0 * d0 + r1 * d1) + r2 * d2;
                const float inv = 1.0f / dl;
                const float e = b[12 + a];
                const float t1 = (-e - ol) * inv, t2 = (e - ol) * inv;
                tmin = fmaxf(tmin, fminf(t1, t2));
                tmax = fminf(tmax, fmaxf(t1, t2));
            }
            if (tmin <= tmax) {
                const int n = cnt < max_hits ? cnt : max_hits;
                int pos = n;
                while (pos > 0 && hit_t[(r * max_hits + pos - 1) * 2] > tmin) --pos;
                if (pos < max_hits) {
                    for (int k = (n < max_hits ? n : max_hits - 1); k > pos; --k) {
                        hit_t[(r * max_hits + k) * 2 + 0] = hit_t[(r * max_hits + k - 1) * 2 + 0];
                        hit_t[(r * max_hits + k) * 2 + 1] = hit_t[(r * max_hits + k - 1) * 2 + 1];
                        hit_box[r * max_hits + k] = hit_box[r * max_hits + k - 1];
                    }
                    hit_t[(r * max_hits + pos) * 2 + 0] = tmin;
                    hit_t[(r * max_hits + pos) * 2 + 1] = tmax;
                    hit_box[r * max_hits + pos] = m;
                }
                ++cnt;
            }
        }
        hit_count[r] = cnt;
    }
}

#define SETUP_MAXH 8
struct RaySetupArgs {
    const float* rays; int64_t R; const float* box; int M; int max_hits; const int32_t* box_ids;
    int N, lindisp, hull; const float* t_rand;
    float* hit_t; int32_t* hit_box; int32_t* hit_count; float* z; int32_t* label_sem; int32_t* label_inst;
};
template <class... Rng>
__global__ __launch_bounds__(256) void k_ray_setup(const RaySetupArgs a, const Rng... rng)
{
    constexpr bool RNG = sizeof...(Rng) > 0;
    __shared__ float2 s_t[SETUP_MAXH][64];
    __shared__ float s_nr[64], s_fr[64];
    __shared__ int s_hb[SETUP_MAXH][64], s_cnt[64];
    const int tid = threadIdx.x, lane = tid & 63, wv = tid >> 6;
    const int mh = a.max_hits, N = a.N;
    PnrRngKey key;
    if constexpr (RNG) key = pnr_rng_key(rng...);
    for (int64_t base = (int64_t)blockIdx.x * 64; base < a.R; base += (int64_t)gridDim.x * 64) {
        const int64_t r = base + tid;
        if (tid < 64 && r < a.R) {
            const float4 ra = *reinterpret_cast<const float4*>(a.rays + r * 8), rb = *reinterpret_cast<const float4*>(a.rays + r * 8 + 4);
            const float o0 = ra.x, o1 = ra.y, o2 = ra.z, d0 = ra.w, d1 = rb.x, d2 = rb.y;
            float nr = rb.z, fr = rb.w;
            for (int h = 0; h < SETUP_MAXH; ++h) { s_hb[h][tid] = -1; s_t[h][tid] = make_float2(0.0f, 0.0f); }
            int cnt = 0;
            for (int m = 0; m < a.M; ++m) {
                const float* b = a.box + m * 15;
                const float p0 = o0 - b[0], p1 = o1 - b[1], p2 = o2 - b[2];
                float tmin = nr, tmax = fr;
#pragma unroll
                for (int x = 0; x < 3; ++x) {
                    const float r0 = b[3 + 3 * x], r1 = b[4 + 3 * x], r2 = b[5 + 3 * x];
                    const float ol = (r0 * p0 + r1 * p1) + r2 * p2;
                    const float dl = (r0 * d0 + r1 * d1) + r2 * d2;
                    const float inv = 1.0f / dl;
                    const float e = b[12 + x];
                    const float t1 = (-e - ol) * inv, t2 = (e - ol) * inv;
                    tmin = fmaxf(tmin, fminf(t1, t2));
                    tmax = fminf(tmax, fmaxf(t1, t2));
                }
                if (tmin <= tmax) {
                    const int n = cnt < mh ? cnt : mh;
                    int pos = n;
                    while (pos > 0 && s_t[pos - 1][tid].x > tmin) --pos;
                    if (pos < mh) {
                        for (int k = (n < mh ? n : mh - 1); k > pos; --k) {
                            s_t[k][tid] = s_t[k - 1][tid];
                            s_hb[k][tid] = s_hb[k - 1][tid];
                        }
                        s_t[pos][tid] = make_float2(tmin, tmax);
                        s_hb[pos][tid] = m;
                    }
                    ++cnt;
                }
            }
            a.hit_count[r] = cnt;
            const int kept = cnt < mh ? cnt : mh;
            for (int h = 0; h < mh; ++h) {
                *reinterpret_cast<float2*>(a.hit_t + (r * mh + h) * 2) = s_t[h][tid];
                a.hit_box[r * mh + h] = s_hb[h][tid];
            }
            if (a.hull && kept > 0) {
                float lo = s_t[0][tid].x, hi = s_t[0][tid].y;
                for (int h = 1; h < kept; ++h) {
                    lo = fminf(lo, s_t[h][tid].x);
                    hi = fmaxf(hi, s_t[h][tid].y);
                }
                nr = lo; fr = hi;
            }
            s_nr[tid] = nr; s_fr[tid] = fr; s_cnt[tid] = kept;
        }
        __syncthreads();
        constexpr int RU = 2;
        for (int rr = wv * 16; rr < wv * 16 + 16; rr += RU) {
            if (base + rr >= a.R) break;
            float nr[RU], fr[RU];
            int cnt[RU], hb[RU][SETUP_MAXH];
            float2 iv[RU][SETUP_MAXH];
#pragma unroll
            for (int u = 0; u < RU; ++u) {
                const int t = rr + u;
                auto uni = [](float v) { return __int_as_float(__builtin_amdgcn_readfirstlane(__float_as_int(v))); };
                nr[u] = uni(s_nr[t]); fr[u] = uni(s_fr[t]);
                cnt[u] = __builtin_amdgcn_readfirstlane(s_cnt[t]);
#pragma unroll
                for (int h = 0; h < SETUP_MAXH; ++h) {
                    const float2 v = s_t[h][t];
                    iv[u][h] = make_float2(uni(v.x), uni(v.y));
                    hb[u][h] = __builtin_amdgcn_readfirstlane(s_hb[h][t]);
                }
            }
#pragma unroll
            for (int u = 0; u < RU; ++u) {
                const int64_t ray = base + rr + u;
                if (ray >= a.R) break;
                for (int i = lane; i < N; i += 64) {
                    const int64_t s = ray * N + i;
                    float zz;
                    if constexpr (RNG) {
                        const float t = pnr_rng_uniform_at(key, (uint32_t)ray, i);
                        zz = strat_sample(nr[u], fr[u], i, N, a.lindisp, &t);
                    } else {
                        zz = strat_sample(nr[u], fr[u], i, N, a.lindisp, a.t_rand ? a.t_rand + s : nullptr);
                    }
                    a.z[s] = zz;
                    if (a.label_sem) {
                        int best = -1, m = -1;
                        float bt = 0.0f;
#pragma unroll
                        for (int h = 0; h < SETUP_MAXH; ++h) {
                            if (h >= cnt[u]) break;
                            const float ti = iv[u][h].x, to = iv[u][h].y;
                            if (ti <= zz && zz <= to && (best < 0 || ti < bt)) { best = h; bt = ti; m = hb[u][h]; }
                        }
                        int ls = -1, li = -1;
                        if (best >= 0) {
                            ls = a.box_ids[m * 2];
                            li = a.box_ids[m * 2 + 1];
                        }
                        a.label_sem[s] = ls;
                        a.label_inst[s] = li;
                    }
                }
            }
        }
        __syncthreads();
    }
}

__global__ __launch_bounds__(256) void k_sample_labels(const float* __restrict__ z, int64_t R, int N,
                                                        const float* __restrict__ hit_t,
                                                        const int32_t* __restrict__ hit_box,
                                                        const int32_t* __restrict__ hit_count, int max_hits,
                                                        const int32_t* __restrict__ box_ids,
                                                        int32_t* __restrict__ label_sem,
                                                        int32_t* __restrict__ label_inst)
{
    const int64_t total = R * N;
    for (int64_t s = (int64_t)blockIdx.x * blockDim.x + threadIdx.x; s < total;
         s += (int64_t)gridDim.x * blockDim.x) {
        const int64_t r = s / N;
        const float zz = z[s];
        const int cnt = hit_count[r] < max_hits ? hit_count[r] : max_hits;
        const int best = label_hit(zz, cnt, [&](int h, float& ti, float& to) {
            ti = hit_t[(r * max_hits + h) * 2];
            to = hit_t[(r * max_hits + h) * 2 + 1];
        });
        int ls = -1, li = -1;
        if (best >= 0) {
            const int m = hit_box[r * max_hits + best];
            ls = box_ids[m * 2];
            li = box_ids[m * 2 + 1];
        }
        label_sem[s] = ls;
        label_inst[s] = li;
    }
}

PNR_EXPORT int pnr_stratified(const float* rays, int64_t n_rays, int n_samples, int lindisp,
                              const float* t_rand, float* z_out, void* stream)
{
    PNR_REQUIRE(n_rays >= 0 && n_samples >= 1, "pnr_stratified: bad size R=%lld N=%d", (long long)n_rays, n_samples);
    if (n_rays == 0) return PNR_OK;
    PNR_REQUIRE(rays && z_out, "pnr_stratified: null pointer");
    const int64_t total = n_rays * n_samples;
    hipLaunchKernelGGL(k_stratified<>, dim3(pnr_grid_cap((total + 255) / 256)), dim3(256), 0, (hipStream_t)stream,
                       rays, n_rays, n_samples, lindisp, t_rand, z_out);
    PNR_CHECK_LAUNCH("pnr_stratified");
    return PNR_OK;
}

PNR_EXPORT int pnr_stratified_rng(const float* rays, int64_t n_rays, int n_samples, int lindisp, const pnr_rng* rng_host,
                                  float* z_out, void* stream)
{
    PnrRngDev rng;
    const int rc = pnr_rng_check(rng_host, n_rays, "pnr_stratified_rng", &rng);
    if (rc) return rc;
    PNR_REQUIRE(n_rays >= 0 && n_samples >= 1 && n_samples <= (1 << 26), "pnr_stratified_rng: bad size R=%lld N=%d", (long long)n_rays,
                n_samples);
    if (n_rays == 0) return PNR_OK;
    PNR_REQUIRE(rays && z_out, "pnr_stratified_rng: null pointer");
    const int64_t total = n_rays * n_samples;
    hipLaunchKernelGGL(k_stratified<PnrRngDev>, dim3(pnr_grid_cap((total + 255) / 256)), dim3(256), 0, (hipStream_t)stream,
                       rays, n_rays, n_samples, lindisp, (const float*)nullptr, z_out, rng);
    PNR_CHECK_LAUNCH("pnr_stratified_rng");
    return PNR_OK;
}

PNR_EXPORT int pnr_points(const float* rays, const float* z, int64_t n_rays, int n_samples, float* pts_out,
                          void* stream)
{
    PNR_REQUIRE(n_rays >= 0 && n_samples >= 1, "pnr_points: bad size");
    if (n_rays == 0) return PNR_OK;
    PNR_REQUIRE(rays && z && pts_out, "pnr_points: null pointer");
    const int64_t total = n_rays * n_samples * 3;
    hipLaunchKernelGGL(k_points, dim3(pnr_grid_cap((total + 255) / 256)), dim3(256), 0, (hipStream_t)stream,
                       rays, z, n_rays, n_samples, pts_out);
    PNR_CHECK_LAUNCH("pnr_points");
    return PNR_OK;
}

PNR_EXPORT int pnr_embed(const float* x, int64_t n, int L, float* out, void* stream)
{
    PNR_REQUIRE(n >= 0 && L >= 0 && L <= 16, "pnr_embed: bad size n=%lld L=%d", (long long)n, L);
    if (n == 0) return PNR_OK;
    PNR_REQUIRE(x && out, "pnr_embed: null pointer");
    const int64_t total = n * (3 + 6 * L);
    hipLaunchKernelGGL(k_embed, dim3(pnr_grid_cap((total + 255) / 256)), dim3(256), 0, (hipStream_t)stream,
                       x, n, L, out);
    PNR_CHECK_LAUNCH("pnr_embed");
    return PNR_OK;
}

static void launch_sample_pdf_rng(const float* z, const float* weights, const PnrRngDev& rng, int64_t n_rays, int n_coarse, int n_fine,
                                  float* z_samples, int32_t* inds, float* z_fine, const PdfLabelArgs& lab, hipStream_t st)
{
    int P = 1;
    while (P < n_coarse + n_fine) P <<= 1;
    if (n_coarse <= 64 && P <= 256)
        hipLaunchKernelGGL(k_sample_pdf_rng, dim3(pnr_grid_cap(n_rays, 32)), dim3(64), 0, st, z, weights, n_rays, n_coarse, n_fine,
                           z_samples, inds, z_fine, lab, rng);
    else
        hipLaunchKernelGGL(k_sample_pdf_big_rng, dim3(pnr_grid_cap(n_rays, 32)), dim3(64), 0, st, z, weights, n_rays, n_coarse, n_fine,
                           z_samples, inds, z_fine, lab, rng);
}

static void launch_sample_pdf(const float* z, const float* weights, const float* u, int64_t n_rays, int n_coarse, int n_fine,
                              float* z_samples, int32_t* inds, float* z_fine, const PdfLabelArgs& lab, hipStream_t st)
{
    int P = 1;
    while (P < n_coarse + n_fine) P <<= 1;
    const bool general_only = getenv("PNR_SAMPLE_PDF_GENERAL") != nullptr;
    if (!u && !z_samples && !inds && z_fine && n_coarse <= 64 && n_fine <= 192 && P <= 256 && lab.max_hits <= 64 && !general_only)
        hipLaunchKernelGGL(k_sample_pdf_det, dim3(pnr_grid_cap(n_rays, 32)), dim3(64), 0, st, z, weights, n_rays, n_coarse, n_fine, z_fine, lab);
    else if (n_coarse <= 64 && P <= 256)
        hipLaunchKernelGGL(k_sample_pdf, dim3(pnr_grid_cap(n_rays, 32)), dim3(64), 0, st, z, weights, u, n_rays, n_coarse, n_fine,
                           z_samples, inds, z_fine, lab);
    else
        hipLaunchKernelGGL(k_sample_pdf_big, dim3(pnr_grid_cap(n_rays, 32)), dim3(64), 0, st, z, weights, u, n_rays, n_coarse,
                           n_fine, z_samples, inds, z_fine, lab);
}

PNR_EXPORT int pnr_sample_pdf(const float* z, const float* weights, const float* u, int64_t n_rays, int n_coarse,
                              int n_fine, float* z_samples, int32_t* inds, float* z_fine, void* stream)
{
    PNR_REQUIRE(n_rays <= 0 || (z && weights), "pnr_sample_pdf: null pointer");
    PNR_REQUIRE(n_coarse >= 3 && n_coarse <= PDF_MAXC, "pnr_sample_pdf: n_coarse=%d outside [3,%d]", n_coarse, PDF_MAXC);
    PNR_REQUIRE(n_fine >= 1 && n_coarse + n_fine <= PDF_MAXT, "pnr_sample_pdf: n_coarse+n_fine=%d > %d",
                n_coarse + n_fine, PDF_MAXT);
    if (n_rays <= 0) return PNR_OK;
    PdfLabelArgs lab;
    memset(&lab, 0, sizeof(lab));
    launch_sample_pdf(z, weights, u, n_rays, n_coarse, n_fine, z_samples, inds, z_fine, lab, (hipStream_t)stream);
    PNR_CHECK_LAUNCH("pnr_sample_pdf");
    return PNR_OK;
}

PNR_EXPORT int pnr_sample_pdf_rng(const float* z, const float* weights, const pnr_rng* rng_host, int64_t n_rays, int n_coarse,
                                  int n_fine, float* z_samples, int32_t* inds, float* z_fine, void* stream)
{
    PnrRngDev rng;
    const int rc = pnr_rng_check(rng_host, n_rays < 0 ? 0 : n_rays, "pnr_sample_pdf_rng", &rng);
    if (rc) return rc;
    PNR_REQUIRE(n_rays <= 0 || (z && weights), "pnr_sample_pdf_rng: null pointer");
    PNR_REQUIRE(n_coarse >= 3 && n_coarse <= PDF_MAXC, "pnr_sample_pdf_rng: n_coarse=%d outside [3,%d]", n_coarse, PDF_MAXC);
    PNR_REQUIRE(n_fine >= 1 && n_coarse + n_fine <= PDF_MAXT, "pnr_sample_pdf_rng: n_coarse+n_fine=%d > %d", n_coarse + n_fine, PDF_MAXT);
    if (n_rays <= 0) return PNR_OK;
    PdfLabelArgs lab;
    memset(&lab, 0, sizeof(lab));
    launch_sample_pdf_rng(z, weights, rng, n_rays, n_coarse, n_fine, z_samples, inds, z_fine, lab, (hipStream_t)stream);
    PNR_CHECK_LAUNCH("pnr_sample_pdf_rng");
    return PNR_OK;
}

PNR_EXPORT int pnr_sample_pdf_labels_rng(const float* z, const float* weights, const pnr_rng* rng_host, int64_t n_rays, int n_coarse,
                                         int n_fine, float* z_fine, const float* hit_t, const int32_t* hit_box, const int32_t* hit_count,
                                         int max_hits, const int32_t* box_ids, int32_t* label_sem, int32_t* label_inst, void* stream)
{
    PnrRngDev rng;
    const int rc = pnr_rng_check(rng_host, n_rays < 0 ? 0 : n_rays, "pnr_sample_pdf_labels_rng", &rng);
    if (rc) return rc;
    PNR_REQUIRE(n_rays <= 0 || (z && weights && z_fine), "pnr_sample_pdf_labels_rng: null pointer");
    PNR_REQUIRE(n_rays <= 0 || (hit_t && hit_box && hit_count && box_ids && label_sem && label_inst), "pnr_sample_pdf_labels_rng: null pointer");
    PNR_REQUIRE(n_coarse >= 3 && n_coarse <= PDF_MAXC, "pnr_sample_pdf_labels_rng: n_coarse=%d outside [3,%d]", n_coarse, PDF_MAXC);
    PNR_REQUIRE(n_fine >= 1 && n_coarse + n_fine <= PDF_MAXT, "pnr_sample_pdf_labels_rng: n_coarse+n_fine=%d > %d", n_coarse + n_fine,
                PDF_MAXT);
    PNR_REQUIRE(max_hits >= 1, "pnr_sample_pdf_labels_rng: bad max_hits");
    if (n_rays <= 0) return PNR_OK;
    PdfLabelArgs lab;
    lab.hit_t = hit_t; lab.hit_box = hit_box; lab.hit_count = hit_count; lab.max_hits = max_hits; lab.box_ids = box_ids;
    lab.label_sem = label_sem; lab.label_inst = label_inst;
    launch_sample_pdf_rng(z, weights, rng, n_rays, n_coarse, n_fine, nullptr, nullptr, z_fine, lab, (hipStream_t)stream);
    PNR_CHECK_LAUNCH("pnr_sample_pdf_labels_rng");
    return PNR_OK;
}

PNR_EXPORT int pnr_sample_pdf_labels(const float* z, const float* weights, const float* u, int64_t n_rays, int n_coarse, int n_fine,
                                     float* z_fine, const float* hit_t, const int32_t* hit_box, const int32_t* hit_count,
                                     int max_hits, const int32_t* box_ids, int32_t* label_sem, int32_t* label_inst, void* stream)
{
    PNR_REQUIRE(n_rays <= 0 || (z && weights && z_fine), "pnr_sample_pdf_labels: null pointer");
    PNR_REQUIRE(n_rays <= 0 || (hit_t && hit_box && hit_count && box_ids && label_sem && label_inst), "pnr_sample_pdf_labels: null pointer");
    PNR_REQUIRE(n_coarse >= 3 && n_coarse <= PDF_MAXC, "pnr_sample_pdf_labels: n_coarse=%d outside [3,%d]", n_coarse, PDF_MAXC);
    PNR_REQUIRE(n_fine >= 1 && n_coarse + n_fine <= PDF_MAXT, "pnr_sample_pdf_labels: n_coarse+n_fine=%d > %d", n_coarse + n_fine, PDF_MAXT);
    PNR_REQUIRE(max_hits >= 1, "pnr_sample_pdf_labels: bad max_hits");
    if (n_rays <= 0) return PNR_OK;
    PdfLabelArgs lab;
    lab.hit_t = hit_t; lab.hit_box = hit_box; lab.hit_count = hit_count; lab.max_hits = max_hits; lab.box_ids = box_ids;
    lab.label_sem = label_sem; lab.label_inst = label_inst;
    launch_sample_pdf(z, weights, u, n_rays, n_coarse, n_fine, nullptr, nullptr, z_fine, lab, (hipStream_t)stream);
    PNR_CHECK_LAUNCH("pnr_sample_pdf_labels");
    return PNR_OK;
}

static int ray_setup_impl(const float* rays, int64_t n_rays, const float* box, int n_box, int max_hits, const int32_t* box_ids,
                          int n_samples, int lindisp, const float* t_rand, const PnrRngDev* rng, int hull, float* hit_t, int32_t* hit_box,
                          int32_t* hit_count, float* z_out, int32_t* label_sem, int32_t* label_inst, void* stream);

PNR_EXPORT int pnr_ray_setup(const float* rays, int64_t n_rays, const float* box, int n_box, int max_hits, const int32_t* box_ids,
                             int n_samples, int lindisp, const float* t_rand, int hull, float* hit_t, int32_t* hit_box,
                             int32_t* hit_count, float* z_out, int32_t* label_sem, int32_t* label_inst, void* stream)
{
    return ray_setup_impl(rays, n_rays, box, n_box, max_hits, box_ids, n_samples, lindisp, t_rand, nullptr, hull, hit_t, hit_box, hit_count,
                          z_out, label_sem, label_inst, stream);
}

PNR_EXPORT int pnr_ray_setup_rng(const float* rays, int64_t n_rays, const float* box, int n_box, int max_hits, const int32_t* box_ids,
                                 int n_samples, int lindisp, const pnr_rng* rng_host, int hull, float* hit_t, int32_t* hit_box,
                                 int32_t* hit_count, float* z_out, int32_t* label_sem, int32_t* label_inst, void* stream)
{
    PnrRngDev rng;
    const int rc = pnr_rng_check(rng_host, n_rays < 0 ? 0 : n_rays, "pnr_ray_setup_rng", &rng);
    if (rc) return rc;
    PNR_REQUIRE(n_samples <= (1 << 26), "pnr_ray_setup_rng: n_samples=%d > 2^26", n_samples);
    return ray_setup_impl(rays, n_rays, box, n_box, max_hits, box_ids, n_samples, lindisp, nullptr, &rng, hull, hit_t, hit_box, hit_count,
                          z_out, label_sem, label_inst, stream);
}

static int ray_setup_impl(const float* rays, int64_t n_rays, const float* box, int n_box, int max_hits, const int32_t* box_ids,
                          int n_samples, int lindisp, const float* t_rand, const PnrRngDev* rng, int hull, float* hit_t, int32_t* hit_box,
                          int32_t* hit_count, float* z_out, int32_t* label_sem, int32_t* label_inst, void* stream)
{
    PNR_REQUIRE(n_rays >= 0 && n_samples >= 1, "pnr_ray_setup: bad size R=%lld N=%d", (long long)n_rays, n_samples);
    PNR_REQUIRE(max_hits >= 1 && max_hits <= SETUP_MAXH, "pnr_ray_setup: max_hits=%d outside [1,%d] (use the separate entry points)",
                max_hits, SETUP_MAXH);
    PNR_REQUIRE(n_box >= 0 && (n_box == 0 || box), "pnr_ray_setup: bad box table");
    if (n_rays == 0) return PNR_OK;
    PNR_REQUIRE(rays && hit_t && hit_box && hit_count && z_out, "pnr_ray_setup: null pointer");
    PNR_REQUIRE((label_sem != nullptr) == (label_inst != nullptr) && (!label_sem || box_ids || n_box == 0),
                "pnr_ray_setup: labels need both outputs and box_ids");
    PNR_REQUIRE((((uintptr_t)rays) & 15) == 0 && (((uintptr_t)hit_t) & 7) == 0, "pnr_ray_setup: rays must be 16-byte aligned");
    RaySetupArgs a;
    a.rays = rays; a.R = n_rays; a.box = box; a.M = n_box; a.max_hits = max_hits; a.box_ids = box_ids;
    a.N = n_samples; a.lindisp = lindisp; a.hull = hull; a.t_rand = t_rand;
    a.hit_t = hit_t; a.hit_box = hit_box; a.hit_count = hit_count; a.z = z_out; a.label_sem = label_sem; a.label_inst = label_inst;
    if (rng)
        hipLaunchKernelGGL(k_ray_setup<PnrRngDev>, dim3(pnr_grid_cap((n_rays + 63) / 64)), dim3(256), 0, (hipStream_t)stream, a, *rng);
    else
        hipLaunchKernelGGL(k_ray_setup<>, dim3(pnr_grid_cap((n_rays + 63) / 64)), dim3(256), 0, (hipStream_t)stream, a);
    PNR_CHECK_LAUNCH("pnr_ray_setup");
    return PNR_OK;
}

PNR_EXPORT int pnr_bbox_hits(const float* rays, int64_t n_rays, const float* box, int n_box, int max_hits,
                             float* hit_t, int32_t* hit_box, int32_t* hit_count, void* stream)
{
    PNR_REQUIRE(n_rays <= 0 || (rays && hit_t && hit_box && hit_count), "pnr_bbox_hits: null pointer");
    PNR_REQUIRE(n_box >= 0 && (n_box == 0 || box), "pnr_bbox_hits: bad box table");
    PNR_REQUIRE(max_hits >= 1 && max_hits <= 64, "pnr_bbox_hits: max_hits=%d outside [1,64]", max_hits);
    if (n_rays <= 0) return PNR_OK;
    hipLaunchKernelGGL(k_bbox_hits, dim3(pnr_grid_cap((n_rays + 255) / 256)), dim3(256), 0, (hipStream_t)stream,
                       rays, n_rays, box, n_box, max_hits, hit_t, hit_box, hit_count);
    PNR_CHECK_LAUNCH("pnr_bbox_hits");
    return PNR_OK;
}

PNR_EXPORT int pnr_sample_labels(const float* z, int64_t n_rays, int n_samples, const float* hit_t,
                                 const int32_t* hit_box, const int32_t* hit_count, int max_hits,
                                 const int32_t* box_ids, int32_t* label_sem, int32_t* label_inst, void* stream)
{
    PNR_REQUIRE(n_rays <= 0 || (z && hit_t && hit_box && hit_count && box_ids && label_sem && label_inst),
                "pnr_sample_labels: null pointer");
    PNR_REQUIRE(n_samples >= 1 && max_hits >= 1, "pnr_sample_labels: bad size");
    if (n_rays <= 0) return PNR_OK;
    const int64_t total = n_rays * n_samples;
    hipLaunchKernelGGL(k_sample_labels, dim3(pnr_grid_cap((total + 255) / 256)), dim3(256), 0,
                       (hipStream_t)stream, z, n_rays, n_samples, hit_t, hit_box, hit_count, max_hits, box_ids,
                       label_sem, label_inst);
    PNR_CHECK_LAUNCH("pnr_sample_labels");
    return PNR_OK;
}

__global__ __launch_bounds__(256) void k_restrict_rays(const float* __restrict__ rays, int64_t R, const float* __restrict__ hit_t,
                                                        const int32_t* __restrict__ hit_count, int max_hits, float* __restrict__ out)
{
    for (int64_t r = (int64_t)blockIdx.x * blockDim.x + threadIdx.x; r < R; r += (int64_t)gridDim.x * blockDim.x) {
        const float4 a = *reinterpret_cast<const float4*>(rays + r * 8);
        float4 b = *reinterpret_cast<const float4*>(rays + r * 8 + 4);
        const int cnt = hit_count[r] < max_hits ? hit_count[r] : max_hits;
        if (cnt > 0) {
            float lo = hit_t[(r * max_hits) * 2], hi = hit_t[(r * max_hits) * 2 + 1];
            for (int h = 1; h < cnt; ++h) {
                lo = fminf(lo, hit_t[(r * max_hits + h) * 2]);
                hi = fmaxf(hi, hit_t[(r * max_hits + h) * 2 + 1]);
            }
            b.z = lo; b.w = hi;
        }
        *reinterpret_cast<float4*>(out + r * 8) = a;
        *reinterpret_cast<float4*>(out + r * 8 + 4) = b;
    }
}

PNR_EXPORT int pnr_restrict_rays(const float* rays, int64_t n_rays, const float* hit_t, const int32_t* hit_count, int max_hits,
                                 float* rays_out, void* stream)
{
    PNR_REQUIRE(n_rays >= 0 && max_hits >= 1, "pnr_restrict_rays: bad size");
    if (n_rays == 0) return PNR_OK;
    PNR_REQUIRE(rays && hit_t && hit_count && rays_out, "pnr_restrict_rays: null pointer");
    PNR_REQUIRE(((((uintptr_t)rays) | ((uintptr_t)rays_out)) & 15) == 0, "pnr_restrict_rays: ray records must be 16-byte aligned");
    hipLaunchKernelGGL(k_restrict_rays, dim3(pnr_grid_cap((n_rays + 255) / 256)), dim3(256), 0, (hipStream_t)stream, rays, n_rays,
                       hit_t, hit_count, max_hits, rays_out);
    PNR_CHECK_LAUNCH("pnr_restrict_rays");
    return PNR_OK;
}
```

### panopticnerf_amd/ops.py

```python
import ctypes
import os

import torch

from . import _lib
from ._lib import MlpDesc, MlpParamsHost


def _stream():
    return ctypes.c_void_p(torch.cuda.current_stream().cuda_stream)


def _chk(t, name, dtype=torch.float32):
    if t is None:
        return None
    if not t.is_cuda:
        raise RuntimeError(f"{name}: expected a GPU tensor (the HIP path has no CPU fallback)")
    if t.dtype != dtype:
        raise TypeError(f"{name}: expected {dtype}, got {t.dtype}")
    if not t.is_contiguous():
        raise ValueError(f"{name}: tensor must be contiguous")
    return t


# ... 846 lines not shown
    if channel_major:
        raw = out if out is not None else alloc_raw(ch, S, z.device)
        ss, sc = 1, _chk_raw(raw, ch, S)
    else:
        raw = out if out is not None else torch.empty((R, N, ch), device=z.device, dtype=torch.float32)
        ss, sc = ch, 1
        _chk(raw, "raw")
    _lib.check(_lib.load().pnr_mlp_forward(ctypes.byref(desc), _p(packed), _p(rays), _p(z), R, N, _p(raw), ss, sc,
                                           _stream()), "pnr_mlp_forward")
    return raw


@_on_device
def composite(raw, z, rays, n_sem=0, n_inst=0, channel_major=True, noise=None, label_sem=None, label_inst=None,
              sem_mode=0, white_bkgd=False, want_weights=True, out=None):
    z, rays = _chk(z, "z"), _chk(rays, "rays")
    draw = noise if _draw(noise) else None
    noise = None if draw is not None else _chk(noise, "noise")
    label_sem = _chk(label_sem, "label_sem", torch.int32)
    label_inst = _chk(label_inst, "label_inst", torch.int32)
    R, N = z.shape
    ch = 4 + n_sem + n_inst
    if channel_major:
        ss, sc = 1, _chk_raw(raw, ch, R * N)
    else:
        _chk(raw, "raw")
        assert tuple(raw.shape) == (R, N, ch)
        ss, sc = ch, 1
    dev = z.device
    out = _maps(out, R, N, n_sem, n_inst, label_sem, label_inst, want_weights, dev)
    g = out.get
    fn, nz, what = _twin("pnr_composite", noise, draw)
    _lib.check(fn(_p(raw), ss, sc, _p(z), _p(rays), nz, _p(label_sem), _p(label_inst), R, N, n_sem, n_inst, int(sem_mode),
                  int(bool(white_bkgd)), _p(out["rgb"]), _p(out["depth"]), _p(out["acc"]), _p(g("weights")), _p(g("semantic")),
                  _p(g("instance")), _p(g("fix_semantic")), _p(g("fix_instance")), _stream()), what)
    return out


def _maps(out, R, N, n_sem, n_inst, label_sem, label_inst, want_weights, dev, drop=()):
    f32 = dict(device=dev, dtype=torch.float32)
    shapes = {"rgb": (R, 3), "depth": (R,), "acc": (R,)}
    if want_weights:
        shapes["weights"] = (R, N)
    if n_sem:
        shapes["semantic"] = (R, n_sem)
        if label_sem is not None:
            shapes["fix_semantic"] = (R, n_sem)
    if n_inst:
        shapes["instance"] = (R, n_inst)
        if label_inst is not None:
            shapes["fix_instance"] = (R, n_inst)
    for k in drop:
        shapes.pop(k, None)
    res = {}
    for k, shp in shapes.items():
        t = out.get(k) if out else None
        if t is None:
            t = torch.empty(shp, **f32)
        elif tuple(t.shape) != shp or t.dtype != torch.float32 or t.device != dev or not t.is_contiguous():
            raise ValueError("out[%r] must be a contiguous fp32 tensor of shape %s on %s" % (k, shp, dev))
        res[k] = t
    return res


def fused_supported(desc, n_samples, sem_mode=0, noise=None):
    ok = (desc.precision == _lib.PREC_BF16 and int(sem_mode) in (0, 1) and noise is None and n_samples % 32 == 0
          and 32 <= n_samples <= 256 and desc.n_sem + desc.n_inst <= 128)
    if ok and int(sem_mode) == 1 and desc.n_sem + desc.n_inst > 0:
        ok = int(_lib.load().pnr_mlp_fused_plan(ctypes.byref(desc_for_mode(desc, 1)))) >= 1
    return ok


def desc_for_mode(desc, sem_mode):
    want = _lib.MLP_SOFTMAX if int(sem_mode) == 1 else 0
    if (desc.flags & _lib.MLP_SOFTMAX) == want:
        return desc
    return _desc_with(desc, flags=(desc.flags & ~_lib.MLP_SOFTMAX) | want)


def fused_image(sem_mode=0):
    return "softmax" if int(sem_mode) == 1 else True


@_on_device
def mlp_forward_composite(desc, packed, rays, z, label_sem=None, label_inst=None, white_bkgd=False, want_weights=True, out=None,
                          sem_mode=0, wg_cap=0):
    rays, z, packed = _chk(rays, "rays"), _chk(z, "z"), _chk(packed, "packed", torch.uint8)
    label_sem = _chk(label_sem, "label_sem", torch.int32)
    label_inst = _chk(label_inst, "label_inst", torch.int32)
    R, N = z.shape
    n_sem, n_inst = desc.n_sem, desc.n_inst
    dev = z.device
    lib = _lib.load()
    desc = desc_for_mode(desc, sem_mode)
    if wg_cap:
        desc = _desc_with(desc, flags=(desc.flags & 0xFFFF) | ((int(wg_cap) & 0x1FF) << 16))
    nbytes = lib.pnr_mlp_forward_composite_workspace_bytes(ctypes.byref(desc), R, N, int(bool(want_weights)))
    if nbytes < 0:
        raise RuntimeError("pnr_mlp_forward_composite: unsupported geometry (n_samples=%d must be a multiple of 32)" % N)
    ws = torch.empty(int(nbytes), device=dev, dtype=torch.uint8)
    out = _maps(out, R, N, n_sem, n_inst, label_sem, label_inst, want_weights, dev)
    g = out.get
    _lib.check(lib.pnr_mlp_forward_composite(ctypes.byref(desc), _p(packed), _p(rays), _p(z), R, N, _p(label_sem), _p(label_inst),
                                             int(bool(white_bkgd)), _p(out["rgb"]), _p(out["depth"]), _p(out["acc"]),
                                             _p(g("weights")), _p(g("semantic")), _p(g("instance")), _p(g("fix_semantic")),
                                             _p(g("fix_instance")), _p(ws), _stream()), "pnr_mlp_forward_composite")
    return out


WEIGHTS_ONLY_DROPS = ("rgb", "semantic", "instance")


def sigma_pass_supported(desc, n_samples, noise=None):
    if not (desc.precision == _lib.PREC_BF16 and noise is None and n_samples % 32 == 0 and 32 <= n_samples <= 256
            and desc.n_sem + desc.n_inst <= 128):
        return False
    return int(_lib.load().pnr_mlp_packed_bytes(ctypes.byref(_desc_with(desc, plan=3)))) > 0


@_on_device
def mlp_forward_weights(desc, packed, rays, z, label_sem=None, label_inst=None, out=None):
    if desc.plan != 3:
        raise ValueError("mlp_forward_weights: needs the plan-3 image (net.packed(level, device, fused='sigma')), not plan %d" % desc.plan)
    rays, z, packed = _chk(rays, "rays"), _chk(z, "z"), _chk(packed, "packed", torch.uint8)
    label_sem = _chk(label_sem, "label_sem", torch.int32)
    label_inst = _chk(label_inst, "label_inst", torch.int32)
    R, N = z.shape
    dev = z.device
    lib = _lib.load()
    nbytes = lib.pnr_mlp_forward_composite_workspace_bytes(ctypes.byref(desc), R, N, 1)
    if nbytes < 0:
        raise RuntimeError("pnr_mlp_forward_composite: unsupported geometry (n_samples=%d must be a multiple of 32)" % N)
    ws = torch.empty(int(nbytes), device=dev, dtype=torch.uint8)
    out = _maps(out, R, N, desc.n_sem, desc.n_inst, label_sem, label_inst, True, dev, drop=WEIGHTS_ONLY_DROPS)
    g = out.get
    _lib.check(lib.pnr_mlp_forward_composite(ctypes.byref(desc), _p(packed), _p(rays), _p(z), R, N, _p(label_sem), _p(label_inst),
                                             0, None, _p(out["depth"]), _p(out["acc"]), _p(out["weights"]), None, None,
                                             _p(g("fix_semantic")), _p(g("fix_instance")), _p(ws), _stream()), "pnr_mlp_forward_composite")
    return out


QUERY_WANTS = ("sigma", "labels", "panoptic", "logits")


def field_query_supported(desc):
    return bool(_lib.load().pnr_mlp_query_supported(ctypes.byref(desc)))


def query_keys(desc, want):
    want = (want,) if isinstance(want, str) else tuple(want)
    bad = [w for w in want if w not in QUERY_WANTS]
    if bad:
        raise ValueError("query: unknown output %r in want (known: %s)" % (bad[0], ", ".join(QUERY_WANTS)))
    keys = []
    if "sigma" in want:
        keys.append("sigma")
    if "labels" in want:
        keys += (["sem_label"] if desc.n_sem else []) + (["inst_label"] if desc.n_inst else [])
    if "panoptic" in want and desc.n_sem:
        keys.append("panoptic")
    if "logits" in want:
        keys += (["sem_logits"] if desc.n_sem else []) + (["inst_logits"] if desc.n_inst else [])
    if not keys:
        raise ValueError("query: want=%r asks for nothing this network has (n_sem=%d, n_inst=%d)" % (want, desc.n_sem, desc.n_inst))
    return keys


@_on_device
def mlp_query(desc, packed, points, want=("sigma", "labels"), is_thing=None, out=None):
    if desc.plan != 4:
        raise ValueError("mlp_query: needs the plan-4 image (net.packed(level, device, fused='field')), not plan %d" % desc.plan)
    keys = query_keys(desc, want)
    points, packed = _chk(points, "points"), _chk(packed, "packed", torch.uint8)
    is_thing = _chk(is_thing, "is_thing", torch.int32)
    if points.dim() != 2 or points.shape[1] != 3:
        raise ValueError("mlp_query: points must be (P, 3), got %s" % (tuple(points.shape),))
    if is_thing is not None and (not desc.n_sem or is_thing.numel() != desc.n_sem):
        raise ValueError("mlp_query: is_thing must hold n_sem=%d entries of a network with a semantic head" % desc.n_sem)
    P, dev = points.shape[0], points.device
    out = dict(out) if out else {}
    res, stride = {}, P
    for k in keys:
        if k.endswith("_logits"):
            n = desc.n_sem if k == "sem_logits" else desc.n_inst
            t = out.get(k)
            if t is None:
                t = alloc_raw(n, P, dev)
            elif (not t.is_cuda or t.dtype != torch.float32 or tuple(t.shape) != (n, P) or (P > 0 and t.stride(1) != 1)
                  or (n > 1 and t.stride(0) < P)):
                raise ValueError("mlp_query: out[%r] must be a float32 GPU tensor of shape %s with unit point stride" % (k, (n, P)))
            res[k] = t
        else:
            res[k] = _own(out.get(k), (P,), torch.float32 if k == "sigma" else torch.int32, dev, "mlp_query: out[%r]" % k)
    lg = [res[k] for k in ("sem_logits", "inst_logits") if k in res]
    if lg:
        stride = lg[0].stride(0) if lg[0].shape[0] > 1 else max(P, lg[0].stride(0))
        if any((t.stride(0) if t.shape[0] > 1 else stride) != stride for t in lg):
            raise ValueError("mlp_query: sem_logits and inst_logits must share one channel stride")
    g = res.get
    _lib.check(_lib.load().pnr_mlp_query(ctypes.byref(desc), _p(packed), _p(points), P, _p(g("sigma")), _p(g("sem_label")),
                                         _p(g("inst_label")), _p(g("panoptic")), _p(is_thing), _p(g("sem_logits")),
                                         _p(g("inst_logits")), stride, _stream()), "pnr_mlp_query")
    return res


@_on_device
def composite_backward(raw, z, rays, n_sem, n_inst, grads, noise=None, label_sem=None, label_inst=None,
                       ce_sem=None, ce_inst=None, sem_mode=0):
    raw, z, rays = _chk(raw, "raw"), _chk(z, "z"), _chk(rays, "rays")
    draw = noise if _draw(noise) else None
    noise = None if draw is not None else _chk(noise, "noise")
    label_sem = _chk(label_sem, "label_sem", torch.int32)
    label_inst = _chk(label_inst, "label_inst", torch.int32)
    R, N = z.shape
    g = {k: _chk(v.contiguous().float(), "g_" + k) for k, v in grads.items() if v is not None}
    ce_sem = None if ce_sem is None else _chk(ce_sem.reshape(1).float().contiguous(), "ce_sem")
    ce_inst = None if ce_inst is None else _chk(ce_inst.reshape(1).float().contiguous(), "ce_inst")
# ... 26 lines not shown
    grads = {k: torch.empty_like(v) for k, v in m.items()} if want_grads else {}
    out = torch.empty(8, device=dev, dtype=torch.float32)
    ws = torch.empty(int(lib.pnr_losses_workspace_bytes(R)), device=dev, dtype=torch.uint8)
    g = grads.get
    _lib.check(lib.pnr_losses(ctypes.byref(cfg), R, int(n_sem), int(n_inst), _p(m.get("rgb")), _p(m.get("depth")),
                              _p(m.get("semantic")), _p(m.get("fix_semantic")), _p(m.get("instance")), _p(m.get("fix_instance")),
                              _p(t_rgb), _p(t_depth), _p(t_sem), _p(t_inst), _p(out), _p(g("rgb")), _p(g("depth")),
                              _p(g("semantic")), _p(g("fix_semantic")), _p(g("instance")), _p(g("fix_instance")), _p(ws),
                              _stream()), "pnr_losses")
    return out, grads


@_on_device
def ce3d(raw, first_channel, n_classes, label):
    lib = _lib.load()
    label = _chk(label, "label", torch.int32)
    S = label.numel()
    sc = _chk_raw(raw, raw.shape[0], S)
    out = torch.empty(2, device=raw.device, dtype=torch.float32)
    ws = torch.empty(int(lib.pnr_ce3d_workspace_bytes(S)), device=raw.device, dtype=torch.uint8)
    _lib.check(lib.pnr_ce3d(_p(raw), sc, int(first_channel), int(n_classes), _p(label), S, _p(out), _p(ws), _stream()), "pnr_ce3d")
    return out


@_on_device
def sample_pdf(z, weights, n_importance, u=None, want_samples=True, out=None):
    z, weights = _chk(z, "z"), _chk(weights, "weights")
    draw = u if _draw(u) else None
    u = None if draw is not None else _chk(u, "u")
    R, Nc = z.shape
    dev = z.device
    z_fine = _own(out, (R, Nc + n_importance), torch.float32, dev, "sample_pdf")
    zs = inds = None
    if want_samples:
        zs = torch.empty((R, n_importance), device=dev, dtype=torch.float32)
        inds = torch.empty((R, n_importance), device=dev, dtype=torch.int32)
    fn, uu, what = _twin("pnr_sample_pdf", u, draw)
    _lib.check(fn(_p(z), _p(weights), uu, R, Nc, n_importance, _p(zs), _p(inds), _p(z_fine), _stream()), what)
    return z_fine, zs, inds


@_on_device
def bbox_hits(rays, box, max_hits=8):
    rays, box = _chk(rays, "rays"), _chk(box, "box")
    R, M = rays.shape[0], box.shape[0]
    dev = rays.device
    hit_t = torch.empty((R, max_hits, 2), device=dev, dtype=torch.float32)
    hit_box = torch.empty((R, max_hits), device=dev, dtype=torch.int32)
    hit_count = torch.empty((R,), device=dev, dtype=torch.int32)
    _lib.check(_lib.load().pnr_bbox_hits(_p(rays), R, _p(box), M, max_hits, _p(hit_t), _p(hit_box), _p(hit_count),
                                         _stream()), "pnr_bbox_hits")
    return hit_t, hit_box, hit_count


@_on_device
def convex_hits(rays, planes, offsets, max_hits=8, out=None):
    rays, planes, offsets = _chk(rays, "rays"), _chk(planes, "planes"), _chk(offsets, "offsets", torch.int32)
    if rays.dim() != 2 or rays.shape[1] != 8:
        raise ValueError("convex_hits: rays must be (R, 8), not %s" % (tuple(rays.shape),))
    if planes.dim() != 2 or planes.shape[1] != 4:
        raise ValueError("convex_hits: planes must be (P, 4), not %s" % (tuple(planes.shape),))
    if offsets.dim() != 1 or offsets.numel() < 1:
        raise ValueError("convex_hits: offsets must be (M + 1,), not %s" % (tuple(offsets.shape),))
    R, M = rays.shape[0], offsets.numel() - 1
    max_hits = int(max_hits)
    if max_hits < 1:
        raise ValueError("convex_hits: max_hits must be >= 1, not %d" % max_hits)
    dev = rays.device
    if planes.shape[0] == 0 and M > 0:
        planes = planes.new_zeros((1, 4))
    o = out if out is not None else (None, None, None)
    hit_t = _own(o[0], (R, max_hits, 2), torch.float32, dev, "convex_hits")
    hit_box = _own(o[1], (R, max_hits), torch.int32, dev, "convex_hits")
    hit_count = _own(o[2], (R,), torch.int32, dev, "convex_hits")
    _lib.check(_lib.load().pnr_convex_hits(_p(rays), R, _p(planes), _p(offsets), M, max_hits, _p(hit_t), _p(hit_box), _p(hit_count),
                                           _stream()), "pnr_convex_hits")
    return hit_t, hit_box, hit_count


RAY_SETUP_MAX_HITS = 8


@_on_device
def ray_setup(rays, box, box_ids=None, n_samples=64, max_hits=8, lindisp=False, t_rand=None, hull=False, out=None):
    rays, box = _chk(rays, "rays"), _chk(box, "box")
    draw = t_rand if _draw(t_rand) else None
    t_rand = None if draw is not None else _chk(t_rand, "t_rand")
    box_ids = _chk(box_ids, "box_ids", torch.int32)
    R, M, N = rays.shape[0], box.shape[0], int(n_samples)
    dev = rays.device
    if t_rand is not None:
        assert tuple(t_rand.shape) == (R, N)
    hit_t = torch.empty((R, max_hits, 2), device=dev, dtype=torch.float32)
    hit_box = torch.empty((R, max_hits), device=dev, dtype=torch.int32)
    hit_count = torch.empty((R,), device=dev, dtype=torch.int32)
    z = _own(out, (R, N), torch.float32, dev, "ray_setup")
    ls = li = None
    if box_ids is not None:
        ls = torch.empty((R, N), device=dev, dtype=torch.int32)
        li = torch.empty((R, N), device=dev, dtype=torch.int32)
    fn, rand, what = _twin("pnr_ray_setup", t_rand, draw)
    _lib.check(fn(_p(rays), R, _p(box), M, int(max_hits), _p(box_ids), N, int(bool(lindisp)), rand, int(bool(hull)), _p(hit_t),
                  _p(hit_box), _p(hit_count), _p(z), _p(ls), _p(li), _stream()), what)
    return (hit_t, hit_box, hit_count), z, ls, li


@_on_device
def sample_pdf_labels(z, weights, n_importance, hits, box_ids, u=None, out=None):
    z, weights = _chk(z, "z"), _chk(weights, "weights")
    draw = u if _draw(u) else None
    u = None if draw is not None else _chk(u, "u")
    hit_t, hit_box, hit_count = _chk(hits[0], "hit_t"), _chk(hits[1], "hit_box", torch.int32), _chk(hits[2], "hit_count", torch.int32)
    box_ids = _chk(box_ids, "box_ids", torch.int32)
    R, Nc = z.shape
    dev = z.device
    Nt = Nc + int(n_importance)
    z_fine = _own(out, (R, Nt), torch.float32, dev, "sample_pdf_labels")
    ls = torch.empty((R, Nt), device=dev, dtype=torch.int32)
    li = torch.empty((R, Nt), device=dev, dtype=torch.int32)
    fn, uu, what = _twin("pnr_sample_pdf_labels", u, draw)
    _lib.check(fn(_p(z), _p(weights), uu, R, Nc, int(n_importance), _p(z_fine), _p(hit_t), _p(hit_box), _p(hit_count), hit_box.shape[1],
                  _p(box_ids), _p(ls), _p(li), _stream()), what)
    return z_fine, ls, li


@_on_device
def restrict_rays(rays, hit_t, hit_count):
    rays = _chk(rays, "rays")
    out = torch.empty_like(rays)
    _lib.check(_lib.load().pnr_restrict_rays(_p(rays), rays.shape[0], _p(_chk(hit_t, "hit_t")), _p(_chk(hit_count, "hit_count", torch.int32)),
                                             hit_t.shape[1], _p(out), _stream()), "pnr_restrict_rays")
    return out


@_on_device
def sample_labels(z, hit_t, hit_box, hit_count, box_ids):
    z, hit_t = _chk(z, "z"), _chk(hit_t, "hit_t")
    hit_box, hit_count = _chk(hit_box, "hit_box", torch.int32), _chk(hit_count, "hit_count", torch.int32)
    box_ids = _chk(box_ids, "box_ids", torch.int32)
    R, N = z.shape
    ls = torch.empty((R, N), device=z.device, dtype=torch.int32)
    li = torch.empty((R, N), device=z.device, dtype=torch.int32)
    _lib.check(_lib.load().pnr_sample_labels(_p(z), R, N, _p(hit_t), _p(hit_box), _p(hit_count), hit_box.shape[1],
                                             _p(box_ids), _p(ls), _p(li), _stream()), "pnr_sample_labels")
    return ls, li


@_on_device
def panoptic_labels(sem, inst=None, is_thing=None):
    sem, inst = _chk(sem, "sem"), _chk(inst, "inst")
    is_thing = _chk(is_thing, "is_thing", torch.int32)
    R, C = sem.shape
    K = inst.shape[1] if inst is not None else 0
    out = [torch.empty(R, device=sem.device, dtype=torch.int32) for _ in range(3)]
    _lib.check(_lib.load().pnr_panoptic_labels(_p(sem), _p(inst), _p(is_thing), R, C, K, _p(out[0]), _p(out[1]), _p(out[2]),
                                               _stream()), "pnr_panoptic_labels")
    return tuple(out)


@_on_device
def confusion(pred, gt, n_classes, conf=None):
    pred, gt = _chk(pred, "pred", torch.int32), _chk(gt, "gt", torch.int32)
    if conf is None:
        conf = torch.zeros((n_classes, n_classes), device=pred.device, dtype=torch.int64)
    _chk(conf, "conf", torch.int64)
    _lib.check(_lib.load().pnr_confusion(_p(pred), _p(gt), pred.numel(), int(n_classes), _p(conf), _stream()), "pnr_confusion")
    return conf
```

### panopticnerf_amd/renderer.py

```python
import collections
import os

import torch

from . import ops


Prims = collections.namedtuple("Prims", "planes offsets")


def _get(cfg, name, default):
    return getattr(cfg, name, default) if cfg is not None else default


CHUNK_QUANTUM = 1024


PREAMBLE_EARLY = os.environ.get("PNR_OVERLAP_PRE", "1") != "0"
CHUNK_TAIL = 8


def chunk_plan(n_rays, chunk_size):
    n_rays, chunk_size = int(n_rays), max(1, int(chunk_size))
    if n_rays <= 0:
        return []
    n = -(-n_rays // chunk_size)
    if n > 1 and n_rays - (n - 1) * chunk_size <= chunk_size // CHUNK_TAIL:
        n -= 1
    size = -(-n_rays // n)
    if n > 1 and chunk_size >= CHUNK_QUANTUM * CHUNK_TAIL:
        size = -(-size // CHUNK_QUANTUM) * CHUNK_QUANTUM
    out, s = [], 0
    while s < n_rays:
        e = min(n_rays, s + size)
        out.append((s, e))
        s = e
    return out


class Renderer:
    def __init__(self, net, cfg=None):
        self.net = net
        self.cfg = cfg
        self.N_samples = _get(cfg, "N_samples", 64)
        self.N_importance = _get(cfg, "N_importance", _get(cfg, "cascade_samples", 0))
        self.chunk_size = _get(cfg, "chunk_size", 65536)
        self.perturb = _get(cfg, "perturb", 0.0)
        self.raw_noise_std = _get(cfg, "raw_noise_std", 0.0)
        self.white_bkgd = _get(cfg, "white_bkgd", False)
        self.lindisp = _get(cfg, "lindisp", False)
        self.max_hits = _get(cfg, "max_hits", 8)
        self.sem_mode = {"none": 0, "logits": 0, "softmax": 1}[_get(cfg, "semantic_activation", "none")]
        self.keep_weights = _get(cfg, "keep_weights", True)
        self.fuse = bool(_get(cfg, "fuse_composite", os.environ.get("PNR_FUSE", "1") != "0"))
        self.strict_hits = bool(_get(cfg, "strict_hits", False))
        self.coarse_outputs = _get(cfg, "coarse_outputs", "all")
        if self.coarse_outputs not in ("all", "weights"):
            raise ValueError("cfg.coarse_outputs must be 'all' or 'weights', not %r" % (self.coarse_outputs,))
        if self.coarse_outputs == "weights" and self.N_importance <= 0:
            raise ValueError("cfg.coarse_outputs = 'weights' needs a fine level (N_importance > 0): without one the coarse maps are "
                             "the render's output")
        self.bbox_sampling = _get(cfg, "bbox_sampling", "none")
        if self.bbox_sampling not in ("none", "hull"):
            raise ValueError("cfg.bbox_sampling must be 'none' or 'hull', not %r" % (self.bbox_sampling,))
        self._overflow = None
        self.rng = _get(cfg, "rng", "torch")
        if self.rng not in ("torch", "device"):
            raise ValueError("cfg.rng must be 'torch' or 'device', not %r" % (self.rng,))
        self.rng_state = None
        if self.rng == "device":
            seed = _get(cfg, "rng_seed", None)
            seed = torch.initial_seed() if seed is None else int(seed)
            seed = (seed + 2 ** 63) % 2 ** 64 - 2 ** 63
            p0 = next(iter(net.parameters()), None)
            self.rng_state = torch.tensor([seed, 0], dtype=torch.int64, device=p0.device if p0 is not None else "cpu")
        self.frame_outputs = bool(_get(cfg, "frame_outputs", os.environ.get("PNR_FRAME_OUT", "1") != "0"))
        self.overlap_levels = bool(_get(cfg, "overlap_levels", os.environ.get("PNR_OVERLAP", "1") != "0"))
        self._side_streams = {}
        if self.N_importance > 0 and getattr(net, "nerf_1", None) is None and not getattr(net, "share_coarse_fine", False):
            raise ValueError("make_renderer: cfg asks for a fine pass (N_importance / cascade_samples = %d) but the network "
                             "was built without a fine NeRF -- build it with make_network(cfg) from the SAME cfg, or set "
                             "cfg.share_coarse_fine = True to evaluate one NeRF at both levels on purpose" % self.N_importance)

    def _preamble(self, rays, box, box_ids, t_rand, z_out):
        hits = lab0 = None
        hull = self.bbox_sampling == "hull"
        prims = isinstance(box, Prims)
        if box is not None and not prims and self.max_hits <= ops.RAY_SETUP_MAX_HITS:
            hits, z, ls0, li0 = ops.ray_setup(rays, box, box_ids, self.N_samples, self.max_hits, self.lindisp, t_rand, hull, out=z_out)
            lab0 = (ls0, li0)
        else:
            if prims:
                hits = ops.convex_hits(rays, box.planes, box.offsets, self.max_hits)
            elif box is not None:
                hits = ops.bbox_hits(rays, box, self.max_hits)
            rays_s = ops.restrict_rays(rays, hits[0], hits[2]) if (hits is not None and hull) else rays
            z = ops.stratified(rays_s, self.N_samples, self.lindisp, t_rand, out=z_out)
        return hits, z, lab0

    def render_rays(self, rays, box=None, box_ids=None, t_rand=None, u=None, train=False, grad=False, out=None, sched=None, rng=None):
        net, Nc, Nf = self.net, self.N_samples, self.N_importance
        n0 = net.nerf(0)
        C, K = n0.n_sem, n0.n_inst
        dev = rays.device
        ret = {}
        hits = lab0 = None
        if t_rand is None and self.perturb > 0 and train:
            t_rand = ops.Draw(rng[0], 1, rng[1]) if rng is not None else torch.rand((rays.shape[0], Nc), device=dev)
        own = (lambda key: out.get(key)) if (out and not grad) else (lambda key: None)
        if sched is not None and sched.get("pre") is not None:
            hits, z, lab0 = sched["pre"]
        else:
            hits, z, lab0 = self._preamble(rays, box, box_ids, t_rand, own("z_vals_0"))
        if hits is not None and self.strict_hits:
            over = torch.stack([(hits[2] > self.max_hits).sum(), hits[2].max()])
            self._overflow = over if self._overflow is None else torch.stack([self._overflow[0] + over[0],
                                                                              torch.maximum(self._overflow[1], over[1])])

        def level(lv, zz, labels=None):
            ls = li = None
            if labels is not None:
                ls, li = labels
            elif hits is not None:
                ls, li = ops.sample_labels(zz, hits[0], hits[1], hits[2], box_ids)
            noise = None
            if self.raw_noise_std > 0 and train:
                if rng is not None:
                    noise = ops.Draw(rng[0], 3 + lv, rng[1], self.raw_noise_std)
                else:
                    noise = torch.randn(zz.shape, device=dev) * self.raw_noise_std
            if grad:
                from . import train as _train
                res = _train.level_train(self, lv, rays, zz, ls, li, noise)
            elif lv == 0 and self.coarse_outputs == "weights":
                mine = {k: own(f"{k}_0") for k in ("depth", "acc", "weights", "fix_semantic", "fix_instance")}
                mine = {k: v for k, v in mine.items() if v is not None}
                if self.fuse and ops.sigma_pass_supported(n0.desc(net.precision), zz.shape[1], noise):
                    desc, img = net.packed(0, dev, fused="sigma")
                    res = ops.mlp_forward_weights(desc, img, rays, zz, ls, li, out=mine)
                else:
                    desc, img = net.packed(0, dev)
                    raw = ops.mlp_forward(desc, img, rays, zz, channel_major=True)
                    res = ops.composite(raw, zz, rays, C, K, True, noise, ls, li, self.sem_mode, self.white_bkgd, True, out=mine)
                    res = {k: v for k, v in res.items() if k not in ops.WEIGHTS_ONLY_DROPS}
            else:
                need_w = self.keep_weights or (lv == 0 and Nf > 0)
                mine = {k: own(f"{k}_{lv}") for k in ("rgb", "depth", "acc", "weights", "semantic", "instance", "fix_semantic", "fix_instance")}
                mine = {k: v for k, v in mine.items() if v is not None}
                if self.fuse and ops.fused_supported(net.nerf(lv).desc(net.precision), zz.shape[1], self.sem_mode, noise):
                    desc, img = net.packed(lv, dev, fused=ops.fused_image(self.sem_mode))
                    if sched is not None and lv == 0 and sched.get("wait") is not None:
                        torch.cuda.current_stream(dev).wait_event(sched["wait"])
                    res = ops.mlp_forward_composite(desc, img, rays, zz, ls, li, self.white_bkgd, need_w, out=mine, sem_mode=self.sem_mode,
                                                    wg_cap=0 if sched is None else sched["caps"][lv])
                else:
                    desc, img = net.packed(lv, dev)
                    raw = ops.mlp_forward(desc, img, rays, zz, channel_major=True)
                    res = ops.composite(raw, zz, rays, C, K, True, noise, ls, li, self.sem_mode, self.white_bkgd, need_w, out=mine)
            for k, v in res.items():
                ret[f"{k}_{lv}"] = v
            ret[f"z_vals_{lv}"] = zz
            return res

        o0 = level(0, z, lab0)
        if Nf > 0:
            if u is None and self.perturb > 0 and train:
                u = ops.Draw(rng[0], 2, rng[1]) if rng is not None else torch.rand((rays.shape[0], Nf), device=dev)
            w0 = o0["weights"].detach().contiguous()
            if hits is not None:
                z_fine, ls1, li1 = ops.sample_pdf_labels(z, w0, Nf, hits, box_ids, u, out=own("z_vals_1"))
                lab1 = (ls1, li1)
            else:
                z_fine, _, _ = ops.sample_pdf(z, w0, Nf, u, want_samples=False, out=own("z_vals_1"))
                lab1 = None
            if sched is not None:
                sched["pdf_done"] = torch.cuda.Event()
                sched["pdf_done"].record(torch.cuda.current_stream(dev))
                if sched.get("before_fine") is not None:
                    sched["before_fine"]()
            level(1, z_fine, lab1)
        return ret

    def _empty_outputs(self, lead, has_box, dev, grad=False):
        n0 = self.net.nerf(0)
        C, K = n0.n_sem, n0.n_inst
        ret = {}
        for lv, N in ((0, self.N_samples),) + (((1, self.N_samples + self.N_importance),) if self.N_importance > 0 else ()):
            need_w = self.keep_weights or (lv == 0 and self.N_importance > 0)
            drop = ops.WEIGHTS_ONLY_DROPS if (lv == 0 and not grad and self.coarse_outputs == "weights") else ()
            m = ops._maps(None, 0, N, C, K, True if has_box else None, True if has_box else None, need_w, dev, drop=drop)
            m["z_vals"] = torch.empty((0, N), device=dev, dtype=torch.float32)
            for k, v in m.items():
                ret[f"{k}_{lv}"] = v.reshape(*lead, *v.shape[1:])
        return ret

    def _overlap_caps(self, dev, plan, grad, train, has_box, t_rand, u):
        if (not self.overlap_levels or grad or train or len(plan) < 2 or not self.fuse or not self.frame_outputs or self.N_importance <= 0
                or self.strict_hits or t_rand is not None or u is not None or self.raw_noise_std > 0 and train
                or self.coarse_outputs == "weights" or torch.cuda.is_current_stream_capturing()):
            return None
        net, Nc, Nt = self.net, self.N_samples, self.N_samples + self.N_importance
        for lv, N in ((0, Nc), (1, Nt)):
            d = net.nerf(lv).desc(net.precision)
            if not ops.fused_supported(d, N, self.sem_mode, None) or net.packed(lv, dev, fused=ops.fused_image(self.sem_mode))[0].plan != 2:
                return None
        cus = torch.cuda.get_device_properties(dev).multi_processor_count
        cap_c = int(round(cus * Nc / float(Nc + Nt) / 8.0)) * 8
        cap_f = cus - cap_c
        if cus % 8 or cap_c < 8 or cap_f < 8 or abs((Nc / float(cap_c)) / (Nt / float(cap_f)) - 1.0) > 0.05:
            return None
        return cap_c, cap_f

    def _frame_maps(self, R, has_box, dev):
        n0 = self.net.nerf(0)
        C, K = n0.n_sem, n0.n_inst
        frame = {}
        for lv, N in ((0, self.N_samples), (1, self.N_samples + self.N_importance)):
            need_w = self.keep_weights or lv == 0
            m = ops._maps(None, R, N, C, K, True if has_box else None, True if has_box else None, need_w, dev)
            m["z_vals"] = torch.empty((R, N), device=dev, dtype=torch.float32)
            for k, v in m.items():
                frame[f"{k}_{lv}"] = v
        return frame

    def _render_overlapped(self, rays, box, box_ids, plan, caps, lead):
        dev = rays.device
        R = rays.shape[0]
        cap_c, cap_f = caps
        frame = self._frame_maps(R, box is not None, dev)
        main = torch.cuda.current_stream(dev)
        if dev not in self._side_streams:
            self._side_streams[dev] = (torch.cuda.Stream(dev), torch.cuda.Stream(dev))
        side = self._side_streams[dev]
        start = torch.cuda.Event()
        start.record(main)
        for st in side:
            st.wait_event(start)
        prev_pdf = None
        pre = {}

        def preamble(cj):
            sj, ej = plan[cj]
            pre[cj] = self._preamble(rays[sj:ej], box, box_ids, None, frame["z_vals_0"][sj:ej])
        for ci, (s, e) in enumerate(plan):
            sched = {"wait": prev_pdf, "caps": (0 if ci == 0 else cap_c, 0 if ci == len(plan) - 1 else cap_f), "pdf_done": None,
                     "pre": pre.pop(ci, None),
                     "before_fine": (lambda cj=ci + 2: preamble(cj)) if (PREAMBLE_EARLY and ci + 2 < len(plan)) else None}
            with torch.cuda.stream(side[ci & 1]):
                o = self.render_rays(rays[s:e], box, box_ids, None, None, False, False, out={k: v[s:e] for k, v in frame.items()}, sched=sched)
                for k, v in o.items():
                    if v.data_ptr() != frame[k][s:e].data_ptr():
                        frame[k][s:e].copy_(v)
            prev_pdf = sched["pdf_done"]
        for st in side:
            done = torch.cuda.Event()
            done.record(st)
            main.wait_event(done)
        return {k: v.reshape(*lead, *v.shape[1:]) for k, v in frame.items()}

    def render(self, batch):
        rays = batch["rays"]
        if not rays.is_cuda:
            raise RuntimeError("Renderer.render: batch['rays'] must be on the GPU (no CPU fallback)")
        grad = torch.is_grad_enabled() and any(p.requires_grad for p in self.net.parameters())
        if grad and self.net.precision not in ("bf16", "fp32"):
            raise ValueError("Renderer.render: precision must be 'bf16' (the training path) or 'fp32' (its parity mode)")
        lead = rays.shape[:-1]
        rays = rays.reshape(-1, 8).float().contiguous()
        R = rays.shape[0]
        box = batch.get("bbox")
        box_ids = batch.get("bbox_ids")
        if batch.get("prim_planes") is not None:
            if box is not None:
                raise ValueError("Renderer.render: the batch has both 'bbox' and 'prim_planes' -- one prior per render: turn the "
                                 "cuboids into primitives with ConvexSet.from_boxes and join the sets with ConvexSet.concat")
            if batch.get("prim_offsets") is None or batch.get("prim_ids") is None:
                raise ValueError("Renderer.render: 'prim_planes' comes with 'prim_offsets' and 'prim_ids' (ConvexSet.batch())")
            box = Prims(batch["prim_planes"].reshape(-1, 4).float().contiguous(), batch["prim_offsets"].reshape(-1).int().contiguous())
            box_ids = batch["prim_ids"].reshape(-1, 2).int().contiguous()
            if box_ids.shape[0] != box.offsets.numel() - 1:
                raise ValueError("Renderer.render: prim_ids has %d rows for %d primitives" % (box_ids.shape[0], box.offsets.numel() - 1))
        elif box is not None:
            box = box.reshape(-1, 15).float().contiguous()
            box_ids = box_ids.reshape(-1, 2).int().contiguous()
        t_rand, u = batch.get("t_rand"), batch.get("u")
        if t_rand is not None:
            t_rand = t_rand.reshape(R, -1).float().contiguous()
        if u is not None:
            u = u.reshape(R, -1).float().contiguous()
        train = self.net.training
        self._overflow = None
        if R == 0:
            return self._empty_outputs(lead, box is not None, rays.device, grad)
        plan = chunk_plan(R, self.chunk_size)
        caps = self._overlap_caps(rays.device, plan, grad, train, box is not None, t_rand, u)
        if caps is not None:
            return self._render_overlapped(rays, box, box_ids, plan, caps, lead)
        call = None
        if self.rng == "device" and train and (self.perturb > 0 or self.raw_noise_std > 0):
            if self.rng_state.device != rays.device:
                self.rng_state = self.rng_state.to(rays.device)
            call = ops.rng_begin(self.rng_state)
        outs = []
        frame = None
        for s, e in plan:
            o = self.render_rays(rays[s:e], box, box_ids,
                                 None if t_rand is None else t_rand[s:e],
                                 None if u is None else u[s:e], train, grad,
                                 out=None if frame is None else {k: v[s:e] for k, v in frame.items()},
                                 rng=None if call is None else (call, s))
            if s == 0 and e < R and not grad and self.frame_outputs and all(v.dim() >= 1 and v.shape[0] == e for v in o.values()):
                frame = {k: torch.empty((R,) + tuple(v.shape[1:]), device=v.device, dtype=v.dtype) for k, v in o.items()}
                for k, v in o.items():
                    frame[k][:e].copy_(v)
            elif frame is not None:
                for k, v in o.items():
                    if v.data_ptr() != frame[k][s:e].data_ptr():
                        frame[k][s:e].copy_(v)
            outs.append(o)
        if self._overflow is not None:
            n_over, worst = (int(v) for v in self._overflow.tolist())
            self._overflow = None
            if n_over > 0:
                raise RuntimeError("Renderer.render: %d ray(s) cross more than max_hits = %d boxes (up to %d): the farthest "
                                   "intervals were dropped -- raise cfg.max_hits" % (n_over, self.max_hits, worst))
        if frame is not None:
# ... 52 lines not shown
```

Before: 1153.

## Pack semantic and instance sample labels into one uint16 per sample

```diff
diff --git a/include/pnr.h b/include/pnr.h
--- a/include/pnr.h
+++ b/include/pnr.h
@@ -40,6 +40,7 @@
 } pnr_mlp_desc;
 
 #define PNR_MLP_SOFTMAX 1
+#define PNR_MLP_LABELS_U16 4
 #define PNR_MLP_WG_CAP(n) (((n) & 0x1FF) << 16)
 #define PNR_MLP_TRACE 0x7A00
 
diff --git a/panopticnerf_amd/_lib.py b/panopticnerf_amd/_lib.py
--- a/panopticnerf_amd/_lib.py
+++ b/panopticnerf_amd/_lib.py
@@ -9,7 +9,7 @@
 c_int = ctypes.c_int
 
 PREC_BF16, PREC_FP32 = 0, 1
-MLP_SOFTMAX, MLP_TRACE = 1, 0x7A00
+MLP_SOFTMAX, MLP_TRACE, MLP_LABELS_U16 = 1, 0x7A00, 4
 CAMERA_PINHOLE, CAMERA_FISHEYE, CAMERA_EQUIRECT = 0, 1, 3
 TAG_PIXEL, TAG_FRAME = 16, 17
 SAMPLE_POOLED, SAMPLE_FRAME = 0, 1
diff --git a/panopticnerf_amd/csrc/pnr_composite.hip b/panopticnerf_amd/csrc/pnr_composite.hip
--- a/panopticnerf_amd/csrc/pnr_composite.hip
+++ b/panopticnerf_amd/csrc/pnr_composite.hip
@@ -327,7 +327,7 @@
     float *rgb, *depth, *acc, *weights, *sem, *inst, *fix_sem, *fix_inst;
 };
 
-template <bool LOGITS>
+template <bool LOGITS, bool U16 = false>
 __global__ __launch_bounds__(256) void k_composite_combine(CombineArgs a)
 {
     __shared__ uint32_t hist_all[4][128];
@@ -338,9 +338,10 @@
     const float* __restrict__ rec = a.rec + ray * T * RF;
     const float4* __restrict__ ps = a.ps + ray * N;
     const float* __restrict__ zr = a.z + ray * N;
-    const bool want_s = a.lab_s && a.fix_sem && C, want_i = a.lab_i && a.fix_inst && K;
+    const bool want_s = a.lab_s && a.fix_sem && C, want_i = (U16 ? a.lab_s : a.lab_i) && a.fix_inst && K;
     const int32_t* __restrict__ lsr = want_s ? a.lab_s + ray * N : nullptr;
     const int32_t* __restrict__ lir = want_i ? a.lab_i + ray * N : nullptr;
+    const uint16_t* __restrict__ lpr = (U16 && (want_s || want_i)) ? reinterpret_cast<const uint16_t*>(a.lab_s) + ray * N : nullptr;
     float q[8];
 #pragma unroll
     for (int k = 0; k < 8; ++k) q[k] = k < T ? rec[k * RF] : 1.0f;
@@ -353,8 +354,14 @@
         const bool in = i < N;
         pv[j] = in ? ps[i] : float4{0.0f, 0.0f, 0.0f, 0.0f};
         zv[j] = in ? zr[i] : 0.0f;
-        lsv[j] = (in && want_s) ? lsr[i] : -1;
-        liv[j] = (in && want_i) ? lir[i] : -1;
+        if constexpr (U16) {
+            const uint32_t b = (in && lpr) ? lpr[i] : 0u;
+            lsv[j] = (int)(b & 0xFFu) - 1;
+            liv[j] = (int)(b >> 8) - 1;
+        } else {
+            lsv[j] = (in && want_s) ? lsr[i] : -1;
+            liv[j] = (in && want_i) ? lir[i] : -1;
+        }
     }
     float lg[2][8];
 #pragma unroll
@@ -417,14 +424,17 @@
 int pnr_composite_combine_launch(const float* rec, int rec_floats, bool logit_sums, const float4* ps, const float* z,
                                  const int32_t* label_sem, const int32_t* label_inst, int64_t R, int N, int C, int K, int white_bkgd,
                                  float* rgb, float* depth, float* acc, float* weights, float* sem, float* inst, float* fix_sem,
-                                 float* fix_inst, hipStream_t st)
+                                 float* fix_inst, hipStream_t st, bool labels_u16)
 {
     CombineArgs a;
     a.rec = rec; a.rec_floats = rec_floats; a.ps = ps; a.z = z; a.lab_s = label_sem; a.lab_i = label_inst;
     a.R = R; a.N = N; a.C = C; a.K = K; a.white_bkgd = white_bkgd;
     a.rgb = rgb; a.depth = depth; a.acc = acc; a.weights = weights; a.sem = sem; a.inst = inst; a.fix_sem = fix_sem; a.fix_inst = fix_inst;
     const int64_t blocks = (R + 3) / 4;
-    if (logit_sums) hipLaunchKernelGGL(k_composite_combine<true>, dim3((unsigned)blocks), dim3(256), 0, st, a);
+    if (labels_u16) {
+        if (logit_sums) hipLaunchKernelGGL((k_composite_combine<true, true>), dim3((unsigned)blocks), dim3(256), 0, st, a);
+        else hipLaunchKernelGGL((k_composite_combine<false, true>), dim3((unsigned)blocks), dim3(256), 0, st, a);
+    } else if (logit_sums) hipLaunchKernelGGL(k_composite_combine<true>, dim3((unsigned)blocks), dim3(256), 0, st, a);
     else hipLaunchKernelGGL(k_composite_combine<false>, dim3((unsigned)blocks), dim3(256), 0, st, a);
     PNR_CHECK_LAUNCH("pnr_mlp_forward_composite (combine)");
     return PNR_OK;
diff --git a/panopticnerf_amd/csrc/pnr_mlp.hip b/panopticnerf_amd/csrc/pnr_mlp.hip
--- a/panopticnerf_amd/csrc/pnr_mlp.hip
+++ b/panopticnerf_amd/csrc/pnr_mlp.hip
@@ -823,7 +823,20 @@
 int pnr_composite_combine_launch(const float* rec, int rec_floats, bool logit_sums, const float4* ps, const float* z,
                                  const int32_t* label_sem, const int32_t* label_inst, int64_t R, int N, int C, int K, int white_bkgd,
                                  float* rgb, float* depth, float* acc, float* weights, float* sem, float* inst, float* fix_sem,
-                                 float* fix_inst, hipStream_t st);
+                                 float* fix_inst, hipStream_t st, bool labels_u16);
+
+static int check_labels(const pnr_mlp_desc* desc, const int32_t* label_sem, const int32_t* label_inst, const float* fix_sem,
+                        const float* fix_inst, const char* who)
+{
+    if (desc && (desc->flags & PNR_MLP_LABELS_U16)) {
+        PNR_REQUIRE((!fix_sem && !fix_inst) || label_sem, "%s: fix_* outputs need the packed labels in label_sem (PNR_MLP_LABELS_U16)", who);
+        PNR_REQUIRE((((uintptr_t)label_sem) & 1) == 0, "%s: packed labels must be 2-byte aligned", who);
+    } else {
+        PNR_REQUIRE((!fix_sem || label_sem) && (!fix_inst || label_inst), "%s: fix_* outputs need their labels (two int32 images; packed "
+                    "uint16 labels need PNR_MLP_LABELS_U16 in desc.flags)", who);
+    }
+    return PNR_OK;
+}
 
 static int record_floats(const pnr_mlp_desc& d)
 {
@@ -936,15 +949,18 @@
     if (n_rays == 0) return PNR_OK;
     PNR_REQUIRE(workspace && z, "pnr_composite_combine: null pointer");
     PNR_REQUIRE(desc->plan != 4, "pnr_composite_combine: a plan-4 (field) image has no compositing workspace");
-    PNR_REQUIRE((!fix_sem || label_sem) && (!fix_inst || label_inst), "pnr_composite_combine: fix_* outputs need their labels");
+    rc = check_labels(desc, label_sem, label_inst, fix_sem, fix_inst, "pnr_composite_combine");
+    if (rc != PNR_OK) return rc;
+    const bool u16 = (desc->flags & PNR_MLP_LABELS_U16) != 0;
     PNR_REQUIRE(desc->plan != 3 || (!rgb && !sem && !inst), "pnr_composite_combine: a plan-3 (sigma-only) workspace has no rgb, semantic "
                 "or instance maps: pass null for them");
     const int rf = record_floats(*desc);
     const int64_t tiles = (n_rays * n_samples + 255) / 256 * 8;
     const float* rec = (const float*)workspace;
-    return pnr_composite_combine_launch(rec, rf, desc->plan != 3, (const float4*)(rec + tiles * rf), z, fix_sem ? label_sem : nullptr,
-                                        fix_inst ? label_inst : nullptr, n_rays, n_samples, desc->n_sem, desc->n_inst, white_bkgd,
-                                        rgb, depth, acc, weights, sem, inst, fix_sem, fix_inst, (hipStream_t)stream);
+    return pnr_composite_combine_launch(rec, rf, desc->plan != 3, (const float4*)(rec + tiles * rf), z,
+                                        (u16 ? (fix_sem || fix_inst) : fix_sem != nullptr) ? label_sem : nullptr,
+                                        fix_inst && !u16 ? label_inst : nullptr, n_rays, n_samples, desc->n_sem, desc->n_inst, white_bkgd,
+                                        rgb, depth, acc, weights, sem, inst, fix_sem, fix_inst, (hipStream_t)stream, u16);
 }
 
 PNR_EXPORT int pnr_mlp_forward_composite(const pnr_mlp_desc* desc, const void* packed, const float* rays, const float* z,
@@ -954,15 +970,18 @@
 {
     PNR_REQUIRE(n_rays >= 0, "pnr_mlp_forward_composite: bad size");
     if (n_rays == 0) return PNR_OK;
-    PNR_REQUIRE((!fix_sem || label_sem) && (!fix_inst || label_inst), "pnr_mlp_forward_composite: fix_* outputs need their labels");
+    int rc = check_labels(desc, label_sem, label_inst, fix_sem, fix_inst, "pnr_mlp_forward_composite");
+    if (rc != PNR_OK) return rc;
     PNR_REQUIRE(!desc || desc->plan != 3 || (!rgb && !sem && !inst), "pnr_mlp_forward_composite: a plan-3 (sigma-only) image has no "
                 "rgb, semantic or instance maps: pass null for them");
     MlpArgs a;
-    int rc = fused_mlp_launch(desc, packed, rays, z, n_rays, n_samples, workspace, stream, a);
+    rc = fused_mlp_launch(desc, packed, rays, z, n_rays, n_samples, workspace, stream, a);
     if (rc != PNR_OK) return rc;
-    return pnr_composite_combine_launch(a.rec, a.rec_floats, desc->plan != 3, a.ps, z, fix_sem ? label_sem : nullptr, fix_inst ? label_inst : nullptr,
-                                        n_rays, n_samples, desc->n_sem, desc->n_inst, white_bkgd, rgb, depth, acc, weights, sem, inst,
-                                        fix_sem, fix_inst, (hipStream_t)stream);
+    const bool u16 = (desc->flags & PNR_MLP_LABELS_U16) != 0;
+    return pnr_composite_combine_launch(a.rec, a.rec_floats, desc->plan != 3, a.ps, z,
+                                        (u16 ? (fix_sem || fix_inst) : fix_sem != nullptr) ? label_sem : nullptr,
+                                        fix_inst && !u16 ? label_inst : nullptr, n_rays, n_samples, desc->n_sem, desc->n_inst, white_bkgd,
+                                        rgb, depth, acc, weights, sem, inst, fix_sem, fix_inst, (hipStream_t)stream, u16);
 }
 
 PNR_EXPORT int pnr_mlp_forward_train(const pnr_mlp_desc* desc, const void* packed, const float* rays, const float* z,
diff --git a/panopticnerf_amd/csrc/pnr_mlp_pack.cpp b/panopticnerf_amd/csrc/pnr_mlp_pack.cpp
--- a/panopticnerf_amd/csrc/pnr_mlp_pack.cpp
+++ b/panopticnerf_amd/csrc/pnr_mlp_pack.cpp
@@ -32,7 +32,7 @@
                 (d->plan == 3 && pnr_plan3_supported(*d)) || (d->plan == 4 && pnr_plan4_supported(*d)),
                 "pnr_mlp: plan=%d is not available for this geometry (ask pnr_mlp_fused_plan; plans 3 and 4: bf16 only)", d->plan);
     const uint32_t trace = (uint32_t)d->flags & 0xFF00u;
-    PNR_REQUIRE(((uint32_t)d->flags & ~(uint32_t)(PNR_MLP_SOFTMAX | 0xFF70u | PNR_MLP_WG_CAP(0x1FF))) == 0 && (trace == 0 || trace == PNR_MLP_TRACE) &&
+    PNR_REQUIRE(((uint32_t)d->flags & ~(uint32_t)(PNR_MLP_SOFTMAX | PNR_MLP_LABELS_U16 | 0xFF70u | PNR_MLP_WG_CAP(0x1FF))) == 0 && (trace == 0 || trace == PNR_MLP_TRACE) &&
                 (trace != 0 || ((uint32_t)d->flags & 0x70u) == 0),
                 "pnr_mlp: unknown bits in flags=0x%x (zero-initialise pnr_mlp_desc; PNR_MLP_* are the defined bits)", (unsigned)d->flags);
     PNR_REQUIRE(((uint32_t)d->clk_probe[0] & 15u) == 0, "pnr_mlp: clk_probe=0x%08x%08x is not a 16-byte aligned device address "
diff --git a/panopticnerf_amd/csrc/pnr_sampling.hip b/panopticnerf_amd/csrc/pnr_sampling.hip
--- a/panopticnerf_amd/csrc/pnr_sampling.hip
+++ b/panopticnerf_amd/csrc/pnr_sampling.hip
@@ -109,6 +109,17 @@
         }
     }
     return best;
+}
+
+__device__ __forceinline__ uint32_t label_byte(int l) { return (0 <= l && l < 255) ? (uint32_t)(l + 1) : 0u; }
+__device__ __forceinline__ void store_labels(int32_t* __restrict__ label_sem, int32_t* __restrict__ label_inst, int64_t s, int ls, int li)
+{
+    if (label_inst) {
+        label_sem[s] = ls;
+        label_inst[s] = li;
+    } else {
+        reinterpret_cast<uint16_t*>(label_sem)[s] = (uint16_t)(label_byte(ls) | (label_byte(li) << 8));
+    }
 }
 
 struct PdfLabelArgs {
@@ -149,8 +160,7 @@
                 ls = lab.box_ids[m * 2];
                 li = lab.box_ids[m * 2 + 1];
             }
-            lab.label_sem[r * Nt + i] = ls;
-            lab.label_inst[r * Nt + i] = li;
+            store_labels(lab.label_sem, lab.label_inst, r * Nt + i, ls, li);
         }
     };
     for (int64_t r = blockIdx.x; r < R; r += gridDim.x) {
@@ -470,10 +480,7 @@
 #pragma unroll
                 for (int k = 0; k < 4; ++k) {
                     const int i = i0 + lane + 64 * k;
-                    if (i < Nt) {
-                        lab.label_sem[r * Nt + i] = ls[k];
-                        lab.label_inst[r * Nt + i] = li[k];
-                    }
+                    if (i < Nt) store_labels(lab.label_sem, lab.label_inst, r * Nt + i, ls[k], li[k]);
                 }
             }
         }
@@ -569,22 +576,28 @@
 __global__ __launch_bounds__(256) void k_ray_setup(const RaySetupArgs a, const Rng... rng)
 {
     constexpr bool RNG = sizeof...(Rng) > 0;
-    __shared__ float2 s_t[SETUP_MAXH][64];
+    __shared__ float2 s_t4[4][SETUP_MAXH][64];
+    __shared__ int s_hb4[4][SETUP_MAXH][64], s_cnt4[4][64];
     __shared__ float s_nr[64], s_fr[64];
-    __shared__ int s_hb[SETUP_MAXH][64], s_cnt[64];
+    __shared__ int s_cnt[64];
+    float2 (*s_t)[64] = s_t4[0];
+    int (*s_hb)[64] = s_hb4[0];
     const int tid = threadIdx.x, lane = tid & 63, wv = tid >> 6;
+    const int wu = __builtin_amdgcn_readfirstlane(wv);
     const int mh = a.max_hits, N = a.N;
     PnrRngKey key;
     if constexpr (RNG) key = pnr_rng_key(rng...);
     for (int64_t base = (int64_t)blockIdx.x * 64; base < a.R; base += (int64_t)gridDim.x * 64) {
-        const int64_t r = base + tid;
-        if (tid < 64 && r < a.R) {
+        const int64_t r = base + lane;
+        float nr = 0.0f, fr = 0.0f;
+        if (r < a.R) {
             const float4 ra = *reinterpret_cast<const float4*>(a.rays + r * 8), rb = *reinterpret_cast<const float4*>(a.rays + r * 8 + 4);
             const float o0 = ra.x, o1 = ra.y, o2 = ra.z, d0 = ra.w, d1 = rb.x, d2 = rb.y;
-            float nr = rb.z, fr = rb.w;
-            for (int h = 0; h < SETUP_MAXH; ++h) { s_hb[h][tid] = -1; s_t[h][tid] = make_float2(0.0f, 0.0f); }
+            nr = rb.z; fr = rb.w;
+            float2 (*w_t)[64] = s_t4[wu];
+            int (*w_hb)[64] = s_hb4[wu];
             int cnt = 0;
-            for (int m = 0; m < a.M; ++m) {
+            for (int m = wu; m < a.M; m += 4) {
                 const float* b = a.box + m * 15;
                 const float p0 = o0 - b[0], p1 = o1 - b[1], p2 = o2 - b[2];
                 float tmin = nr, tmax = fr;
@@ -602,33 +615,77 @@
                 if (tmin <= tmax) {
                     const int n = cnt < mh ? cnt : mh;
                     int pos = n;
-                    while (pos > 0 && s_t[pos - 1][tid].x > tmin) --pos;
+                    while (pos > 0 && w_t[pos - 1][lane].x > tmin) --pos;
                     if (pos < mh) {
                         for (int k = (n < mh ? n : mh - 1); k > pos; --k) {
-                            s_t[k][tid] = s_t[k - 1][tid];
-                            s_hb[k][tid] = s_hb[k - 1][tid];
+                            w_t[k][lane] = w_t[k - 1][lane];
+                            w_hb[k][lane] = w_hb[k - 1][lane];
                         }
-                        s_t[pos][tid] = make_float2(tmin, tmax);
-                        s_hb[pos][tid] = m;
+                        w_t[pos][lane] = make_float2(tmin, tmax);
+                        w_hb[pos][lane] = m;
                     }
                     ++cnt;
                 }
             }
-            a.hit_count[r] = cnt;
-            const int kept = cnt < mh ? cnt : mh;
-            for (int h = 0; h < mh; ++h) {
-                *reinterpret_cast<float2*>(a.hit_t + (r * mh + h) * 2) = s_t[h][tid];
-                a.hit_box[r * mh + h] = s_hb[h][tid];
+            s_cnt4[wu][lane] = cnt;
+        }
+        __syncthreads();
+        if (wu == 0 && r < a.R) {
+            int hd[4], kc[4], cb[4], total = 0;
+            float2 ct[4];
+#pragma unroll
+            for (int w = 0; w < 4; ++w) {
+                const int c = s_cnt4[w][lane];
+                total += c;
+                kc[w] = c < mh ? c : mh;
+                hd[w] = 0;
+                cb[w] = -1;
+                ct[w] = make_float2(0.0f, 0.0f);
+                if (kc[w] > 0) { ct[w] = s_t4[w][0][lane]; cb[w] = s_hb4[w][0][lane]; }
+            }
+            float2 ot[SETUP_MAXH];
+            int ob[SETUP_MAXH];
+#pragma unroll
+            for (int k = 0; k < SETUP_MAXH; ++k) {
+                int bw = -1, bb = -1;
+                float2 bt = make_float2(0.0f, 0.0f);
+                if (k < mh) {
+#pragma unroll
+                    for (int w = 0; w < 4; ++w)
+                        if (cb[w] >= 0 && (bw < 0 || ct[w].x < bt.x || (ct[w].x == bt.x && cb[w] < bb))) { bw = w; bt = ct[w]; bb = cb[w]; }
+#pragma unroll
+                    for (int w = 0; w < 4; ++w)
+                        if (w == bw) {
+                            ++hd[w];
+                            cb[w] = -1;
+                            if (hd[w] < kc[w]) { ct[w] = s_t4[w][hd[w]][lane]; cb[w] = s_hb4[w][hd[w]][lane]; }
+                        }
+                }
+                ot[k] = bt; ob[k] = bb;
+            }
+            a.hit_count[r] = total;
+            const int kept = total < mh ? total : mh;
+#pragma unroll
+            for (int h = 0; h < SETUP_MAXH; ++h) {
+                s_t[h][lane] = ot[h];
+                s_hb[h][lane] = ob[h];
+                if (h < mh) {
+                    *reinterpret_cast<float2*>(a.hit_t + (r * mh + h) * 2) = ot[h];
+                    a.hit_box[r * mh + h] = ob[h];
+                }
             }
             if (a.hull && kept > 0) {
-                float lo = s_t[0][tid].x, hi = s_t[0][tid].y;
-                for (int h = 1; h < kept; ++h) {
-                    lo = fminf(lo, s_t[h][tid].x);
-                    hi = fmaxf(hi, s_t[h][tid].y);
+                float lo = ot[0].x, hi = ot[0].y;
+#pragma unroll
+                for (int h = 1; h < SETUP_MAXH; ++h) {
+                    if (h < kept) {
+                        lo = fminf(lo, ot[h].x);
+                        hi = fmaxf(hi, ot[h].y);
+                    }
                 }
                 nr = lo; fr = hi;
             }
-            s_nr[tid] = nr; s_fr[tid] = fr; s_cnt[tid] = kept;
+            s_nr[lane] = nr; s_fr[lane] = fr; s_cnt[lane] = kept;
         }
         __syncthreads();
         constexpr int RU = 2;
@@ -678,8 +735,7 @@
                             ls = a.box_ids[m * 2];
                             li = a.box_ids[m * 2 + 1];
                         }
-                        a.label_sem[s] = ls;
-                        a.label_inst[s] = li;
+                        store_labels(a.label_sem, a.label_inst, s, ls, li);
                     }
                 }
             }
@@ -712,8 +768,7 @@
             ls = box_ids[m * 2];
             li = box_ids[m * 2 + 1];
         }
-        label_sem[s] = ls;
-        label_inst[s] = li;
+        store_labels(label_sem, label_inst, s, ls, li);
     }
 }
 
@@ -842,6 +897,7 @@
     if (rc) return rc;
     PNR_REQUIRE(n_rays <= 0 || (z && weights && z_fine), "pnr_sample_pdf_labels_rng: null pointer");
     PNR_REQUIRE(n_rays <= 0 || (hit_t && hit_box && hit_count && box_ids && label_sem && label_inst), "pnr_sample_pdf_labels_rng: null pointer");
+    PNR_REQUIRE(label_inst != label_sem || (((uintptr_t)label_sem) & 1) == 0, "pnr_sample_pdf_labels_rng: packed labels must be 2-byte aligned");
     PNR_REQUIRE(n_coarse >= 3 && n_coarse <= PDF_MAXC, "pnr_sample_pdf_labels_rng: n_coarse=%d outside [3,%d]", n_coarse, PDF_MAXC);
     PNR_REQUIRE(n_fine >= 1 && n_coarse + n_fine <= PDF_MAXT, "pnr_sample_pdf_labels_rng: n_coarse+n_fine=%d > %d", n_coarse + n_fine,
                 PDF_MAXT);
@@ -849,7 +905,7 @@
     if (n_rays <= 0) return PNR_OK;
     PdfLabelArgs lab;
     lab.hit_t = hit_t; lab.hit_box = hit_box; lab.hit_count = hit_count; lab.max_hits = max_hits; lab.box_ids = box_ids;
-    lab.label_sem = label_sem; lab.label_inst = label_inst;
+    lab.label_sem = label_sem; lab.label_inst = label_inst == label_sem ? nullptr : label_inst;
     launch_sample_pdf_rng(z, weights, rng, n_rays, n_coarse, n_fine, nullptr, nullptr, z_fine, lab, (hipStream_t)stream);
     PNR_CHECK_LAUNCH("pnr_sample_pdf_labels_rng");
     return PNR_OK;
@@ -861,13 +917,14 @@
 {
     PNR_REQUIRE(n_rays <= 0 || (z && weights && z_fine), "pnr_sample_pdf_labels: null pointer");
     PNR_REQUIRE(n_rays <= 0 || (hit_t && hit_box && hit_count && box_ids && label_sem && label_inst), "pnr_sample_pdf_labels: null pointer");
+    PNR_REQUIRE(label_inst != label_sem || (((uintptr_t)label_sem) & 1) == 0, "pnr_sample_pdf_labels: packed labels must be 2-byte aligned");
     PNR_REQUIRE(n_coarse >= 3 && n_coarse <= PDF_MAXC, "pnr_sample_pdf_labels: n_coarse=%d outside [3,%d]", n_coarse, PDF_MAXC);
     PNR_REQUIRE(n_fine >= 1 && n_coarse + n_fine <= PDF_MAXT, "pnr_sample_pdf_labels: n_coarse+n_fine=%d > %d", n_coarse + n_fine, PDF_MAXT);
     PNR_REQUIRE(max_hits >= 1, "pnr_sample_pdf_labels: bad max_hits");
     if (n_rays <= 0) return PNR_OK;
     PdfLabelArgs lab;
     lab.hit_t = hit_t; lab.hit_box = hit_box; lab.hit_count = hit_count; lab.max_hits = max_hits; lab.box_ids = box_ids;
-    lab.label_sem = label_sem; lab.label_inst = label_inst;
+    lab.label_sem = label_sem; lab.label_inst = label_inst == label_sem ? nullptr : label_inst;
     launch_sample_pdf(z, weights, u, n_rays, n_coarse, n_fine, nullptr, nullptr, z_fine, lab, (hipStream_t)stream);
     PNR_CHECK_LAUNCH("pnr_sample_pdf_labels");
     return PNR_OK;
@@ -909,11 +966,13 @@
     PNR_REQUIRE(rays && hit_t && hit_box && hit_count && z_out, "pnr_ray_setup: null pointer");
     PNR_REQUIRE((label_sem != nullptr) == (label_inst != nullptr) && (!label_sem || box_ids || n_box == 0),
                 "pnr_ray_setup: labels need both outputs and box_ids");
+    PNR_REQUIRE(label_inst != label_sem || (((uintptr_t)label_sem) & 1) == 0, "pnr_ray_setup: packed labels must be 2-byte aligned");
     PNR_REQUIRE((((uintptr_t)rays) & 15) == 0 && (((uintptr_t)hit_t) & 7) == 0, "pnr_ray_setup: rays must be 16-byte aligned");
     RaySetupArgs a;
     a.rays = rays; a.R = n_rays; a.box = box; a.M = n_box; a.max_hits = max_hits; a.box_ids = box_ids;
     a.N = n_samples; a.lindisp = lindisp; a.hull = hull; a.t_rand = t_rand;
-    a.hit_t = hit_t; a.hit_box = hit_box; a.hit_count = hit_count; a.z = z_out; a.label_sem = label_sem; a.label_inst = label_inst;
+    a.hit_t = hit_t; a.hit_box = hit_box; a.hit_count = hit_count; a.z = z_out; a.label_sem = label_sem;
+    a.label_inst = label_inst == label_sem ? nullptr : label_inst;
     if (rng)
         hipLaunchKernelGGL(k_ray_setup<PnrRngDev>, dim3(pnr_grid_cap((n_rays + 63) / 64)), dim3(256), 0, (hipStream_t)stream, a, *rng);
     else
@@ -941,12 +1000,13 @@
 {
     PNR_REQUIRE(n_rays <= 0 || (z && hit_t && hit_box && hit_count && box_ids && label_sem && label_inst),
                 "pnr_sample_labels: null pointer");
+    PNR_REQUIRE(label_inst != label_sem || (((uintptr_t)label_sem) & 1) == 0, "pnr_sample_labels: packed labels must be 2-byte aligned");
     PNR_REQUIRE(n_samples >= 1 && max_hits >= 1, "pnr_sample_labels: bad size");
     if (n_rays <= 0) return PNR_OK;
     const int64_t total = n_rays * n_samples;
     hipLaunchKernelGGL(k_sample_labels, dim3(pnr_grid_cap((total + 255) / 256)), dim3(256), 0,
                        (hipStream_t)stream, z, n_rays, n_samples, hit_t, hit_box, hit_count, max_hits, box_ids,
-                       label_sem, label_inst);
+                       label_sem, label_inst == label_sem ? nullptr : label_inst);
     PNR_CHECK_LAUNCH("pnr_sample_labels");
     return PNR_OK;
 }
diff --git a/panopticnerf_amd/ops.py b/panopticnerf_amd/ops.py
--- a/panopticnerf_amd/ops.py
+++ b/panopticnerf_amd/ops.py
@@ -952,13 +952,34 @@
     return "softmax" if int(sem_mode) == 1 else True
 
 
+PACKED_LABEL_DTYPES = (torch.int16, torch.uint16) if hasattr(torch, "uint16") else (torch.int16,)
+
+
+def unpack_labels(packed):
+    w = packed.view(torch.int16).to(torch.int32) & 0xFFFF
+    return (w & 0xFF) - 1, (w >> 8) - 1
+
+
+def _fused_labels(desc, label_sem, label_inst, what):
+    packed = label_sem is not None and label_sem.dtype in PACKED_LABEL_DTYPES
+    if packed:
+        if label_inst is not None:
+            raise ValueError(f"{what}: a packed label tensor carries both fields: pass it as label_sem and leave label_inst None")
+        label_sem = _chk(label_sem, "label_sem", label_sem.dtype)
+        return _desc_with(desc, flags=desc.flags | _lib.MLP_LABELS_U16), label_sem, None, True, True
+    if desc.flags & _lib.MLP_LABELS_U16:
+        raise ValueError(f"{what}: desc.flags has PNR_MLP_LABELS_U16 but label_sem is not a packed int16 / uint16 tensor")
+    return desc, _chk(label_sem, "label_sem", torch.int32), _chk(label_inst, "label_inst", torch.int32), label_sem is not None, label_inst is not None
+
+
 @_on_device
 def mlp_forward_composite(desc, packed, rays, z, label_sem=None, label_inst=None, white_bkgd=False, want_weights=True, out=None,
                           sem_mode=0, wg_cap=0):
     rays, z, packed = _chk(rays, "rays"), _chk(z, "z"), _chk(packed, "packed", torch.uint8)
-    label_sem = _chk(label_sem, "label_sem", torch.int32)
-    label_inst = _chk(label_inst, "label_inst", torch.int32)
+    desc, label_sem, label_inst, has_s, has_i = _fused_labels(desc, label_sem, label_inst, "mlp_forward_composite")
     R, N = z.shape
+    if label_sem is not None and tuple(label_sem.shape) != (R, N):
+        raise ValueError("mlp_forward_composite: label_sem must have z's shape %s, not %s" % ((R, N), tuple(label_sem.shape)))
     n_sem, n_inst = desc.n_sem, desc.n_inst
     dev = z.device
     lib = _lib.load()
@@ -969,7 +990,7 @@
     if nbytes < 0:
         raise RuntimeError("pnr_mlp_forward_composite: unsupported geometry (n_samples=%d must be a multiple of 32)" % N)
     ws = torch.empty(int(nbytes), device=dev, dtype=torch.uint8)
-    out = _maps(out, R, N, n_sem, n_inst, label_sem, label_inst, want_weights, dev)
+    out = _maps(out, R, N, n_sem, n_inst, True if has_s else None, True if has_i else None, want_weights, dev)
     g = out.get
     _lib.check(lib.pnr_mlp_forward_composite(ctypes.byref(desc), _p(packed), _p(rays), _p(z), R, N, _p(label_sem), _p(label_inst),
                                              int(bool(white_bkgd)), _p(out["rgb"]), _p(out["depth"]), _p(out["acc"]),
@@ -993,16 +1014,17 @@
     if desc.plan != 3:
         raise ValueError("mlp_forward_weights: needs the plan-3 image (net.packed(level, device, fused='sigma')), not plan %d" % desc.plan)
     rays, z, packed = _chk(rays, "rays"), _chk(z, "z"), _chk(packed, "packed", torch.uint8)
-    label_sem = _chk(label_sem, "label_sem", torch.int32)
-    label_inst = _chk(label_inst, "label_inst", torch.int32)
+    desc, label_sem, label_inst, has_s, has_i = _fused_labels(desc, label_sem, label_inst, "mlp_forward_weights")
     R, N = z.shape
+    if label_sem is not None and tuple(label_sem.shape) != (R, N):
+        raise ValueError("mlp_forward_weights: label_sem must have z's shape %s, not %s" % ((R, N), tuple(label_sem.shape)))
     dev = z.device
     lib = _lib.load()
     nbytes = lib.pnr_mlp_forward_composite_workspace_bytes(ctypes.byref(desc), R, N, 1)
     if nbytes < 0:
         raise RuntimeError("pnr_mlp_forward_composite: unsupported geometry (n_samples=%d must be a multiple of 32)" % N)
     ws = torch.empty(int(nbytes), device=dev, dtype=torch.uint8)
-    out = _maps(out, R, N, desc.n_sem, desc.n_inst, label_sem, label_inst, True, dev, drop=WEIGHTS_ONLY_DROPS)
+    out = _maps(out, R, N, desc.n_sem, desc.n_inst, True if has_s else None, True if has_i else None, True, dev, drop=WEIGHTS_ONLY_DROPS)
     g = out.get
     _lib.check(lib.pnr_mlp_forward_composite(ctypes.byref(desc), _p(packed), _p(rays), _p(z), R, N, _p(label_sem), _p(label_inst),
                                              0, None, _p(out["depth"]), _p(out["acc"]), _p(out["weights"]), None, None,
@@ -1195,7 +1217,7 @@
 
 
 @_on_device
-def ray_setup(rays, box, box_ids=None, n_samples=64, max_hits=8, lindisp=False, t_rand=None, hull=False, out=None):
+def ray_setup(rays, box, box_ids=None, n_samples=64, max_hits=8, lindisp=False, t_rand=None, hull=False, out=None, packed=False):
     rays, box = _chk(rays, "rays"), _chk(box, "box")
     draw = t_rand if _draw(t_rand) else None
     t_rand = None if draw is not None else _chk(t_rand, "t_rand")
@@ -1210,16 +1232,18 @@
     z = _own(out, (R, N), torch.float32, dev, "ray_setup")
     ls = li = None
     if box_ids is not None:
-        ls = torch.empty((R, N), device=dev, dtype=torch.int32)
-        li = torch.empty((R, N), device=dev, dtype=torch.int32)
+        ls = torch.empty((R, N), device=dev, dtype=torch.int16 if packed else torch.int32)
+        li = None if packed else torch.empty((R, N), device=dev, dtype=torch.int32)
     fn, rand, what = _twin("pnr_ray_setup", t_rand, draw)
     _lib.check(fn(_p(rays), R, _p(box), M, int(max_hits), _p(box_ids), N, int(bool(lindisp)), rand, int(bool(hull)), _p(hit_t),
-                  _p(hit_box), _p(hit_count), _p(z), _p(ls), _p(li), _stream()), what)
+                  _p(hit_box), _p(hit_count), _p(z), _p(ls), _p(ls if packed else li), _stream()), what)
+    if packed:
+        return (hit_t, hit_box, hit_count), z, ls
     return (hit_t, hit_box, hit_count), z, ls, li
 
 
 @_on_device
-def sample_pdf_labels(z, weights, n_importance, hits, box_ids, u=None, out=None):
+def sample_pdf_labels(z, weights, n_importance, hits, box_ids, u=None, out=None, packed=False):
     z, weights = _chk(z, "z"), _chk(weights, "weights")
     draw = u if _draw(u) else None
     u = None if draw is not None else _chk(u, "u")
@@ -1229,11 +1253,13 @@
     dev = z.device
     Nt = Nc + int(n_importance)
     z_fine = _own(out, (R, Nt), torch.float32, dev, "sample_pdf_labels")
-    ls = torch.empty((R, Nt), device=dev, dtype=torch.int32)
-    li = torch.empty((R, Nt), device=dev, dtype=torch.int32)
+    ls = torch.empty((R, Nt), device=dev, dtype=torch.int16 if packed else torch.int32)
+    li = None if packed else torch.empty((R, Nt), device=dev, dtype=torch.int32)
     fn, uu, what = _twin("pnr_sample_pdf_labels", u, draw)
     _lib.check(fn(_p(z), _p(weights), uu, R, Nc, int(n_importance), _p(z_fine), _p(hit_t), _p(hit_box), _p(hit_count), hit_box.shape[1],
-                  _p(box_ids), _p(ls), _p(li), _stream()), what)
+                  _p(box_ids), _p(ls), _p(ls if packed else li), _stream()), what)
+    if packed:
+        return z_fine, ls
     return z_fine, ls, li
 
 
@@ -1247,16 +1273,16 @@
 
 
 @_on_device
-def sample_labels(z, hit_t, hit_box, hit_count, box_ids):
+def sample_labels(z, hit_t, hit_box, hit_count, box_ids, packed=False):
     z, hit_t = _chk(z, "z"), _chk(hit_t, "hit_t")
     hit_box, hit_count = _chk(hit_box, "hit_box", torch.int32), _chk(hit_count, "hit_count", torch.int32)
     box_ids = _chk(box_ids, "box_ids", torch.int32)
     R, N = z.shape
-    ls = torch.empty((R, N), device=z.device, dtype=torch.int32)
-    li = torch.empty((R, N), device=z.device, dtype=torch.int32)
+    ls = torch.empty((R, N), device=z.device, dtype=torch.int16 if packed else torch.int32)
+    li = None if packed else torch.empty((R, N), device=z.device, dtype=torch.int32)
     _lib.check(_lib.load().pnr_sample_labels(_p(z), R, N, _p(hit_t), _p(hit_box), _p(hit_count), hit_box.shape[1],
-                                             _p(box_ids), _p(ls), _p(li), _stream()), "pnr_sample_labels")
-    return ls, li
+                                             _p(box_ids), _p(ls), _p(ls if packed else li), _stream()), "pnr_sample_labels")
+    return ls if packed else (ls, li)
 
 
 @_on_device
diff --git a/panopticnerf_amd/renderer.py b/panopticnerf_amd/renderer.py
--- a/panopticnerf_amd/renderer.py
+++ b/panopticnerf_amd/renderer.py
@@ -77,18 +77,31 @@
         self.frame_outputs = bool(_get(cfg, "frame_outputs", os.environ.get("PNR_FRAME_OUT", "1") != "0"))
         self.overlap_levels = bool(_get(cfg, "overlap_levels", os.environ.get("PNR_OVERLAP", "1") != "0"))
         self._side_streams = {}
+        self.packed_labels = bool(_get(cfg, "packed_labels", os.environ.get("PNR_PACKED_LABELS", "1") != "0"))
         if self.N_importance > 0 and getattr(net, "nerf_1", None) is None and not getattr(net, "share_coarse_fine", False):
             raise ValueError("make_renderer: cfg asks for a fine pass (N_importance / cascade_samples = %d) but the network "
                              "was built without a fine NeRF -- build it with make_network(cfg) from the SAME cfg, or set "
                              "cfg.share_coarse_fine = True to evaluate one NeRF at both levels on purpose" % self.N_importance)
 
-    def _preamble(self, rays, box, box_ids, t_rand, z_out):
+    def _packs(self, lv, N, grad=False, train=False):
+        if not self.packed_labels or grad or not self.fuse or (self.raw_noise_std > 0 and train):
+            return False
+        d = self.net.nerf(lv).desc(self.net.precision)
+        if lv == 0 and self.coarse_outputs == "weights":
+            return ops.sigma_pass_supported(d, N, None)
+        return ops.fused_supported(d, N, self.sem_mode, None)
+
+    def _preamble(self, rays, box, box_ids, t_rand, z_out, packed=False):
         hits = lab0 = None
         hull = self.bbox_sampling == "hull"
         prims = isinstance(box, Prims)
         if box is not None and not prims and self.max_hits <= ops.RAY_SETUP_MAX_HITS:
-            hits, z, ls0, li0 = ops.ray_setup(rays, box, box_ids, self.N_samples, self.max_hits, self.lindisp, t_rand, hull, out=z_out)
-            lab0 = (ls0, li0)
+            if packed:
+                hits, z, lp0 = ops.ray_setup(rays, box, box_ids, self.N_samples, self.max_hits, self.lindisp, t_rand, hull, out=z_out, packed=True)
+                lab0 = (lp0, None)
+            else:
+                hits, z, ls0, li0 = ops.ray_setup(rays, box, box_ids, self.N_samples, self.max_hits, self.lindisp, t_rand, hull, out=z_out)
+                lab0 = (ls0, li0)
         else:
             if prims:
                 hits = ops.convex_hits(rays, box.planes, box.offsets, self.max_hits)
@@ -111,7 +124,7 @@
         if sched is not None and sched.get("pre") is not None:
             hits, z, lab0 = sched["pre"]
         else:
-            hits, z, lab0 = self._preamble(rays, box, box_ids, t_rand, own("z_vals_0"))
+            hits, z, lab0 = self._preamble(rays, box, box_ids, t_rand, own("z_vals_0"), self._packs(0, Nc, grad, train))
         if hits is not None and self.strict_hits:
             over = torch.stack([(hits[2] > self.max_hits).sum(), hits[2].max()])
             self._overflow = over if self._overflow is None else torch.stack([self._overflow[0] + over[0],
@@ -121,6 +134,8 @@
             ls = li = None
             if labels is not None:
                 ls, li = labels
+            elif hits is not None and self._packs(lv, zz.shape[1], grad, train):
+                ls = ops.sample_labels(zz, hits[0], hits[1], hits[2], box_ids, packed=True)
             elif hits is not None:
                 ls, li = ops.sample_labels(zz, hits[0], hits[1], hits[2], box_ids)
             noise = None
@@ -168,8 +183,12 @@
                 u = ops.Draw(rng[0], 2, rng[1]) if rng is not None else torch.rand((rays.shape[0], Nf), device=dev)
             w0 = o0["weights"].detach().contiguous()
             if hits is not None:
-                z_fine, ls1, li1 = ops.sample_pdf_labels(z, w0, Nf, hits, box_ids, u, out=own("z_vals_1"))
-                lab1 = (ls1, li1)
+                if self._packs(1, Nc + Nf, grad, train):
+                    z_fine, lp1 = ops.sample_pdf_labels(z, w0, Nf, hits, box_ids, u, out=own("z_vals_1"), packed=True)
+                    lab1 = (lp1, None)
+                else:
+                    z_fine, ls1, li1 = ops.sample_pdf_labels(z, w0, Nf, hits, box_ids, u, out=own("z_vals_1"))
+                    lab1 = (ls1, li1)
             else:
                 z_fine, _, _ = ops.sample_pdf(z, w0, Nf, u, want_samples=False, out=own("z_vals_1"))
                 lab1 = None
@@ -241,7 +260,7 @@
 
         def preamble(cj):
             sj, ej = plan[cj]
-            pre[cj] = self._preamble(rays[sj:ej], box, box_ids, None, frame["z_vals_0"][sj:ej])
+            pre[cj] = self._preamble(rays[sj:ej], box, box_ids, None, frame["z_vals_0"][sj:ej], self._packs(0, self.N_samples))
         for ci, (s, e) in enumerate(plan):
             sched = {"wait": prev_pdf, "caps": (0 if ci == 0 else cap_c, 0 if ci == len(plan) - 1 else cap_f), "pdf_done": None,
                      "pre": pre.pop(ci, None),
```

After: 1155, median of 6. About the same (+0.2%).
